# zeromq/jeromq

Hardware: AMD Instinct MI355X
Metric: CURVE encrypt+MAC GiB/s (device-resident), batched 4 KiB frames, 1/2/4/8 GPU (higher is better)
Workload: dtype u32; 1 GPU; 1M x 4 KiB frames, seal (configs[1]); frames_per_gpu=1048576, payload_bytes_per_gpu=4294967296, parallelism=shard1

## Files before the change

### jeromq_amd/build.py

```python
import os
import shutil
import struct
import subprocess
import sys
import tempfile
from concurrent.futures import ThreadPoolExecutor

HERE = os.path.dirname(os.path.abspath(__file__))
ROOT = os.path.dirname(HERE)
CSRC = os.path.join(HERE, "csrc")
PRODUCT_LIB = os.path.join(HERE, "libcurvezmq_mi355x.so")
LIB = os.environ.get("CZ_LIB_OUT", PRODUCT_LIB)
SOURCES = ["cz_kernels.hip#1", "cz_kernels.hip#2", "cz_kernels.hip#3", "cz_x25519.hip", "cz_host.cpp", "cz_mechanism.cpp", "cz_wire.cpp", "cz_engine.cpp", "cz_handshake.cpp", "cz_curve_hs.cpp", "cz_hs_parse.cpp", "cz_acceptor.cpp", "cz_connector.cpp"]
HEADERS = ["cz_accept.h", "cz_accept_kernels.h", "cz_connect.h", "cz_connect_kernels.h", "cz_hs_batch.h", "cz_hs_dev.h",
           "cz_hs_records.h", "cz_hs_parse.h", "cz_device.h", "cz_fe25519.h", "cz_diag.h", "cz_dispatch.h", "cz_internal.h", "cz_launch.h", "cz_salsa_lazy.h", "cz_salsa_tail.h", "cz_session.h", os.path.join("..", "..", "include", "curvezmq_mi355x.h")]
ARCH = os.environ.get("CZ_OFFLOAD_ARCH", "gfx950")
LLVM_BIN = "/opt/rocm/lib/llvm/bin"
BUNDLE_MAGIC = b"__CLANG_OFFLOAD_BUNDLE__"


class IsaHazardError(RuntimeError):
    pass


class ProductFlagsError(ValueError):
    """Extra compile flags (A/B variants, wrong-output diagnostics) asked for the product library."""


def compile_flags(lib, extra_env=None):
    raw = os.environ.get("CZ_EXTRA_FLAGS", "") if extra_env is None else extra_env
    extra = raw.split()
    product = os.path.realpath(lib) == os.path.realpath(PRODUCT_LIB)
    if product and extra:
        raise ProductFlagsError(f"CZ_EXTRA_FLAGS={raw!r} refused for the product library {PRODUCT_LIB}: "
                                "A/B builds set CZ_LIB_OUT to another path")
    common = [f"--offload-arch={ARCH}", "-O3", "-std=c++17", "-fPIC", "-Wall"]
    return common + (["-DCZ_PRODUCT_BUILD"] if product else extra)


def _stale(lib=LIB, sources=SOURCES):
    if not os.path.exists(lib):
        return True
    t = os.path.getmtime(lib)
    return any(os.path.getmtime(os.path.join(CSRC, f.split("#")[0])) > t for f in list(sources) + HEADERS)


def device_code_objects(so_path, arch=ARCH):
    with tempfile.TemporaryDirectory() as td:
        fb = os.path.join(td, "fatbin")
        subprocess.run([os.path.join(LLVM_BIN, "llvm-objcopy"), "--dump-section", f".hip_fatbin={fb}", so_path,
                        os.path.join(td, "discard")], check=True, capture_output=True)
        data = open(fb, "rb").read()
    cos, i = [], data.find(BUNDLE_MAGIC)
    while i >= 0:
        (n,) = struct.unpack_from("<Q", data, i + len(BUNDLE_MAGIC))
        p = i + len(BUNDLE_MAGIC) + 8
        for _ in range(n):
            off, size, tlen = struct.unpack_from("<QQQ", data, p)
            triple = data[p + 24:p + 24 + tlen].decode()
            p += 24 + tlen
            if triple.endswith("--" + arch) and size:
                cos.append(data[i + off:i + off + size])
        i = data.find(BUNDLE_MAGIC, i + 1)
    return cos


def _elf_functions(co):
    (shoff,) = struct.unpack_from("<Q", co, 0x28)
    shentsize, shnum = struct.unpack_from("<HH", co, 0x3A)
    secs = [struct.unpack_from("<IIQQQQIIQQ", co, shoff + k * shentsize) for k in range(shnum)]
    out = []
    for sec in secs:
        if sec[1] != 2:
            continue
        strtab = secs[sec[6]]
        for k in range(sec[5] // 24):
            name_off, info, _, shndx, value, size = struct.unpack_from("<IBBHQQ", co, sec[4] + 24 * k)
            if info & 0xF != 2 or not size or shndx >= len(secs):
                continue
            end = co.index(b"\0", strtab[4] + name_off)
            name = co[strtab[4] + name_off:end].decode()
            text = secs[shndx]
            start = text[4] + (value - text[3])
            out.append((name, bytes(co[start:start + size])))
    return out


def kernel_code_sha256(so_path, kernels, arch=ARCH):
    import hashlib
    funcs = [f for co in device_code_objects(so_path, arch) for f in _elf_functions(co)]
    names = [n for n, _ in funcs]
    filt = shutil.which("c++filt") or shutil.which("llvm-cxxfilt")
    dem = subprocess.run([filt], input="\n".join(names), capture_output=True, text=True, check=True).stdout.split("\n")
    code = {}
    for (n, b), d in zip(funcs, dem):
        d = d.replace("(anonymous namespace)::", "")
        code.setdefault(d.split("(")[0].replace("void ", "", 1).strip(), b)
    h = hashlib.sha256()
    for k in sorted(kernels):
        if k not in code:
            return None
        h.update(k.encode() + b"\0" + code[k])
    return h.hexdigest()


def disassemble(code_object, arch=ARCH):
    with tempfile.NamedTemporaryFile(suffix=".co") as f:
        f.write(code_object)
        f.flush()
        out = subprocess.run([os.path.join(LLVM_BIN, "llvm-objdump"), "-d", f"--mcpu={arch}", f.name],
                             check=True, capture_output=True, text=True).stdout
    lines = []
    for ln in out.splitlines():
        ln = ln.split("//")[0].rstrip()
        if ln.strip() and not ln.endswith(":") and not ln.startswith(("Disassembly", "/")):
            lines.append(ln)
    return "\n".join(lines)


def isa_gate(so_path, arch=ARCH):
    sys.path.insert(0, os.path.join(ROOT, "tools"))
    from isa_store_hazard import scan
    cos = device_code_objects(so_path, arch)
    if not cos:
        raise IsaHazardError(f"{so_path}: no {arch} code object found to scan")
    total, hits = 0, []
    for co in cos:
        text = disassemble(co, arch)
        total += text.count("\n") + 1
        d, s, r = scan(text)
        hits += [("store data rewritten at distance 1", x) for x in d]
        hits += [("VALU-written SGPR read by VMEM within 5 states", x) for x in s]
        hits += [("wide buffer store with a register soffset", x) for x in r]
    if hits:
        raise IsaHazardError(f"{so_path}: {len(hits)} VMEM store hazard(s) in the {arch} ISA, "
                             f"library not installed; first: {hits[:3]}")
    return len(cos), total


def build_library(force=False, verbose=True, sources=None, lib=None, src_dir=None, jobs=None):
    sources = list(sources or SOURCES)
    lib = lib or LIB
    src_dir = src_dir or CSRC
    compile_flags(lib)
    if not force and src_dir == CSRC and not _stale(lib, sources):
        return lib
    hipcc = os.environ.get("HIPCC", "/opt/rocm/bin/hipcc")
    common = compile_flags(lib)
    objdir = tempfile.mkdtemp(prefix="cz_build_")
    try:
        def compile_one(entry):
            f, _, part = entry.partition("#")
            obj = os.path.join(objdir, os.path.splitext(f)[0] + (f"_{part}" if part else "") + ".o")
            cmd = [hipcc] + common + ([f"-DCZ_KPART={part}"] if part else []) + ["-c", "-o", obj, os.path.join(src_dir, f)]
            if verbose:
                print(" ".join(cmd), file=sys.stderr)
            r = subprocess.run(cmd, cwd=src_dir, capture_output=True, text=True)
            if r.returncode:
                errs = [ln for ln in r.stderr.splitlines() if "error" in ln][:20]
                print("\n".join(errs), file=sys.stderr)
                raise subprocess.CalledProcessError(r.returncode, cmd, r.stdout, r.stderr)
            return obj
        order = sorted(sources, key=lambda f: -os.path.getsize(os.path.join(src_dir, f.split("#")[0])))
        with ThreadPoolExecutor(max_workers=jobs or min(len(order), os.cpu_count() or 4, 8)) as ex:
            objs = list(ex.map(compile_one, order))
        tmp = f"{lib}.{os.getpid()}.tmp"
        subprocess.check_call([hipcc, f"--offload-arch={ARCH}", "-shared", "-fPIC", "-o", tmp] + objs, cwd=src_dir)
        try:
            n_co, n_ins = isa_gate(tmp)
        except Exception:
            os.unlink(tmp)
            raise
        if verbose:
            print(f"isa gate: {n_co} {ARCH} code objects, {n_ins} instructions, 0 store hazards", file=sys.stderr)
        os.replace(tmp, lib)
    finally:
        shutil.rmtree(objdir, ignore_errors=True)
    return lib


JNI_DIR = os.path.join(ROOT, "jni")
JNI_BENCH = os.path.join(ROOT, "tools", "bin", "jni_bench")
JNI_WRAPPED = ("cz_box_afternm", "cz_box_open_afternm", "cz_secretbox", "cz_secretbox_open", "cz_box_beforenm", "cz_box",
               "cz_box_open", "cz_box_keypair", "cz_engine_add_conn")


def build_jni_bench(lib=PRODUCT_LIB, out=JNI_BENCH):
    os.makedirs(os.path.dirname(out), exist_ok=True)
    rel = os.path.relpath(os.path.dirname(lib), os.path.dirname(out))
    cmd = ["gcc", "-std=c11", "-O2", "-Wall", "-Wextra", "-Werror", "-DCZ_JNI_MIN", "-I" + JNI_DIR,
           "-I" + os.path.join(ROOT, "include"), os.path.join(JNI_DIR, "jni_bench.c"),
           os.path.join(JNI_DIR, "curvezmq_jni.c"), os.path.join(JNI_DIR, "fake_jni_env.c"),
           "-L" + os.path.dirname(lib), "-lcurvezmq_mi355x", "-Wl,-rpath,$ORIGIN/" + rel,
           "-Wl," + ",".join("--wrap=" + f for f in JNI_WRAPPED), "-o", out]
    subprocess.check_call(cmd)
    return out


if __name__ == "__main__":
    build_library(force="--force" in sys.argv)
    print(LIB)
```

### jeromq_amd/csrc/cz_device.h

```cpp
#pragma once
#include <hip/hip_runtime.h>
#include <stdint.h>

#include "cz_salsa_lazy.h"
#include "cz_salsa_tail.h"

namespace cz {

typedef uint32_t u32;
typedef uint64_t u64;

constexpr u32 SIGMA0 = 0x61707865u, SIGMA1 = 0x3320646eu, SIGMA2 = 0x79622d32u, SIGMA3 = 0x6b206574u;

__device__ __forceinline__ u32 rotl(u32 v, int c) { return __builtin_amdgcn_alignbit(v, v, 32 - c); }

__device__ __forceinline__ void qr(u32 &a, u32 &b, u32 &c, u32 &d)
{
    b ^= rotl(a + d, 7);
    c ^= rotl(b + a, 9);
    d ^= rotl(c + b, 13);
    a ^= rotl(d + c, 18);
}

__device__ __forceinline__ void col_round(u32 x[16])
{
    qr(x[0], x[4], x[8], x[12]);
    qr(x[5], x[9], x[13], x[1]);
    qr(x[10], x[14], x[2], x[6]);
    qr(x[15], x[3], x[7], x[11]);
}

__device__ __forceinline__ void row_round(u32 x[16])
{
    qr(x[0], x[1], x[2], x[3]);
    qr(x[5], x[6], x[7], x[4]);
    qr(x[10], x[11], x[8], x[9]);
    qr(x[15], x[12], x[13], x[14]);
}

template <int C>
__device__ __forceinline__ u32 srotl(u32 v)
{
    u32 r, t;
    asm("s_lshl_b32 %0, %2, %3\n\ts_lshr_b32 %1, %2, %4\n\ts_or_b32 %0, %0, %1"
        : "=&s"(r), "=&s"(t)
        : "s"(v), "i"(C), "i"(32 - C)
        : "scc");
    return r;
}

struct SalsaFrame {
    u32 w[16];
};

__device__ __forceinline__ SalsaFrame salsa_frame(const u32 k[8], u32 n0, u32 n1)
{
    u32 x[16] = {SIGMA0, k[0], k[1], k[2], k[3], SIGMA1, n0, n1, 0u, 0u, SIGMA2, k[4], k[5], k[6], k[7], SIGMA3};
    x[9] ^= srotl<7>(x[5] + x[1]);   x[13] ^= srotl<9>(x[9] + x[5]);
    x[1] ^= srotl<13>(x[13] + x[9]); x[5] ^= srotl<18>(x[1] + x[13]);
    x[14] ^= srotl<7>(x[10] + x[6]); x[2] ^= srotl<9>(x[14] + x[10]);
    x[6] ^= srotl<13>(x[2] + x[14]); x[10] ^= srotl<18>(x[6] + x[2]);
    x[3] ^= srotl<7>(x[15] + x[11]); x[7] ^= srotl<9>(x[3] + x[15]);
    x[11] ^= rotl(x[7] + x[3], 13);  x[15] ^= rotl(x[11] + x[7], 18);
    SalsaFrame f;
#pragma unroll
    for (int i = 0; i < 16; i++)
        f.w[i] = x[i];
    return f;
}

__device__ __forceinline__ void rounds12_frame(u32 x[16], const SalsaFrame &f, u32 c0, const u32 k[8])
{
#pragma unroll
    for (int i = 0; i < 16; i++)
        x[i] = f.w[i];
    x[0] = SIGMA0; x[4] = k[3]; x[8] = c0; x[12] = k[5];
    x[4] ^= srotl<7>(x[0] + x[12]);  x[8] ^= srotl<9>(x[4] + x[0]);
    x[12] ^= srotl<13>(x[8] + x[4]); x[0] ^= srotl<18>(x[12] + x[8]);
    x[1] ^= srotl<7>(x[0] + x[3]);   x[2] ^= srotl<9>(x[1] + x[0]);
    x[3] ^= srotl<13>(x[2] + x[1]);  x[0] ^= srotl<18>(x[3] + x[2]);
    x[6] ^= srotl<7>(x[5] + x[4]);   x[7] ^= srotl<9>(x[6] + x[5]);
    x[4] ^= rotl(x[7] + x[6], 13);   x[5] ^= rotl(x[4] + x[7], 18);
    x[11] ^= rotl(x[10] + x[9], 7);  x[8] ^= rotl(x[11] + x[10], 9);
    x[9] ^= rotl(x[8] + x[11], 13);  x[10] ^= rotl(x[9] + x[8], 18);
    x[12] ^= rotl(x[15] + x[14], 7); x[13] ^= rotl(x[12] + x[15], 9);
    x[14] ^= rotl(x[13] + x[12], 13); x[15] ^= rotl(x[14] + x[13], 18);
}

static_assert(CZ_LAZY_FIRST_ROUND == 3, "rounds_lazy runs rounds 1-2 in C");
template <bool R12 = false>
__device__ __forceinline__ void rounds_lazy(u32 x[16], u32 d[16])
{
    if constexpr (!R12) {
        col_round(x);
        row_round(x);
    }
    u32 t0, t1, t2, t3;
    asm(CZ_SALSA_LAZY_ASM
        : "+v"(x[0]), "+v"(x[1]), "+v"(x[2]), "+v"(x[3]), "+v"(x[4]), "+v"(x[5]), "+v"(x[6]), "+v"(x[7]),
          "+v"(x[8]), "+v"(x[9]), "+v"(x[10]), "+v"(x[11]), "+v"(x[12]), "+v"(x[13]), "+v"(x[14]), "+v"(x[15]),
          "=&v"(d[0]), "=&v"(d[1]), "=&v"(d[2]), "=&v"(d[3]), "=&v"(d[4]), "=&v"(d[5]), "=&v"(d[6]), "=&v"(d[7]),
          "=&v"(d[8]), "=&v"(d[9]), "=&v"(d[10]), "=&v"(d[11]), "=&v"(d[12]), "=&v"(d[13]), "=&v"(d[14]),
          "=&v"(d[15]), "=&v"(t0), "=&v"(t1), "=&v"(t2), "=&v"(t3));
}

__device__ __forceinline__ constexpr bool lazy_pending(int k) { return (CZ_LAZY_PENDING >> k) & 1u; }

__device__ __forceinline__ void rounds_eager(u32 x[16])
{
#pragma unroll
    for (int i = 0; i < 10; i++) {
        col_round(x);
        row_round(x);
    }
}

template <bool LAZY = true>
__device__ __forceinline__ void salsa20_block(u32 x[16], const u32 k[8], u32 n0, u32 n1, u32 c0, u32 c1)
{
    const u32 in[16] = {SIGMA0, k[0], k[1], k[2], k[3], SIGMA1, n0, n1, c0, c1, SIGMA2, k[4], k[5], k[6], k[7], SIGMA3};
#pragma unroll
    for (int i = 0; i < 16; i++)
        x[i] = in[i];
    if constexpr (LAZY) {
        u32 d[16];
        rounds_lazy(x, d);
#pragma unroll
        for (int i = 0; i < 16; i++)
            x[i] = lazy_pending(i) ? ((x[i] ^ d[i]) + in[i]) : (x[i] + in[i]);
    } else {
        rounds_eager(x);
#pragma unroll
        for (int i = 0; i < 16; i++)
            x[i] += in[i];
    }
}

__device__ __forceinline__ void salsa20_block_frame(u32 x[16], const SalsaFrame &f, const u32 k[8], u32 n0, u32 n1,
                                                    u32 c0)
{
    const u32 in[16] = {SIGMA0, k[0], k[1], k[2], k[3], SIGMA1, n0, n1, c0, 0u, SIGMA2, k[4], k[5], k[6], k[7], SIGMA3};
    u32 d[16];
    rounds12_frame(x, f, c0, k);
    rounds_lazy<true>(x, d);
#pragma unroll
    for (int i = 0; i < 16; i++)
        x[i] = lazy_pending(i) ? ((x[i] ^ d[i]) + in[i]) : (x[i] + in[i]);
}

__device__ __forceinline__ void tail_lazy(u32 x[16], u32 d[16])
{
    u32 t0, t1, t2, t3;
    asm(CZ_SALSA_TAIL_ASM
        : "+v"(x[0]), "+v"(x[1]), "+v"(x[2]), "+v"(x[3]), "+v"(x[4]), "+v"(x[5]), "+v"(x[6]), "+v"(x[7]),
          "+v"(x[8]), "+v"(x[9]), "+v"(x[10]), "+v"(x[11]), "+v"(x[12]), "+v"(x[13]), "+v"(x[14]), "+v"(x[15]),
          "=&v"(d[0]), "=&v"(d[1]), "=&v"(d[2]), "=&v"(d[3]), "=&v"(d[4]), "=&v"(d[5]), "=&v"(d[6]), "=&v"(d[7]),
          "=&v"(d[8]), "=&v"(d[9]), "=&v"(d[10]), "=&v"(d[11]), "=&v"(d[12]), "=&v"(d[13]), "=&v"(d[14]),
          "=&v"(d[15]), "=&v"(t0), "=&v"(t1), "=&v"(t2), "=&v"(t3));
}
static_assert(CZ_SALSA_TAIL_WORDS == 4, "tail blocks use keystream words 0..3");

template <bool LAZY = true>
__device__ __forceinline__ void salsa20_block_w03(u32 x[16], const u32 k[8], u32 n0, u32 n1, u32 c0, u32 c1)
{
    const u32 in[16] = {SIGMA0, k[0], k[1], k[2], k[3], SIGMA1, n0, n1, c0, c1, SIGMA2, k[4], k[5], k[6], k[7], SIGMA3};
#pragma unroll
    for (int i = 0; i < 16; i++)
        x[i] = in[i];
    if constexpr (LAZY) {
        u32 d[16];
        col_round(x);
        row_round(x);
        tail_lazy(x, d);
#pragma unroll
        for (int i = 0; i < 4; i++)
            x[i] = lazy_pending(i) ? ((x[i] ^ d[i]) + in[i]) : (x[i] + in[i]);
    } else {
        rounds_eager(x);
#pragma unroll
        for (int i = 0; i < 4; i++)
            x[i] += in[i];
    }
}

__device__ __forceinline__ void salsa20_block_frame_w03(u32 x[16], const SalsaFrame &f, const u32 k[8], u32 n0, u32 n1,
                                                        u32 c0)
{
    const u32 in[4] = {SIGMA0, k[0], k[1], k[2]};
    u32 d[16];
    rounds12_frame(x, f, c0, k);
    tail_lazy(x, d);
#pragma unroll
    for (int i = 0; i < 4; i++)
        x[i] = lazy_pending(i) ? ((x[i] ^ d[i]) + in[i]) : (x[i] + in[i]);
    (void)n0, (void)n1;
}

__device__ __forceinline__ void hsalsa20(u32 out[8], const u32 k[8], const u32 in[4])
{
    u32 x[16], d[16];
    x[0] = SIGMA0; x[1] = k[0]; x[2] = k[1]; x[3] = k[2];
    x[4] = k[3]; x[5] = SIGMA1; x[6] = in[0]; x[7] = in[1];
    x[8] = in[2]; x[9] = in[3]; x[10] = SIGMA2; x[11] = k[4];
    x[12] = k[5]; x[13] = k[6]; x[14] = k[7]; x[15] = SIGMA3;
    rounds_lazy(x, d);
    constexpr int w[8] = {0, 5, 10, 15, 6, 7, 8, 9};
#pragma unroll
    for (int i = 0; i < 8; i++)
        out[i] = lazy_pending(w[i]) ? (x[w[i]] ^ d[w[i]]) : x[w[i]];
}

struct Poly {
    u32 h0, h1, h2, h3, h4;
    u32 r0, r1, r2, r3;
    u32 s1, s2, s3;
    u32 p0, p1, p2, p3;
};

__device__ __forceinline__ void poly_init(Poly &P, u32 k0, u32 k1, u32 k2, u32 k3, u32 k4, u32 k5, u32 k6, u32 k7)
{
    P.r0 = k0 & 0x0fffffffu;
    P.r1 = k1 & 0x0ffffffcu;
    P.r2 = k2 & 0x0ffffffcu;
    P.r3 = k3 & 0x0ffffffcu;
    P.s1 = P.r1 + (P.r1 >> 2);
    P.s2 = P.r2 + (P.r2 >> 2);
    P.s3 = P.r3 + (P.r3 >> 2);
    P.p0 = k4; P.p1 = k5; P.p2 = k6; P.p3 = k7;
    P.h0 = P.h1 = P.h2 = P.h3 = P.h4 = 0;
}

__device__ __forceinline__ u32 addc(u32 a, u32 b, u32 cin, u32 &cout)
{
    return __builtin_addc(a, b, cin, &cout);
}

__device__ __forceinline__ u64 mad64(u32 a, u32 b, u64 c) { return (u64)a * b + c; }

template <bool CIN = false>
__device__ __forceinline__ void poly_block(Poly &P, u32 m0, u32 m1, u32 m2, u32 m3, u32 hibit)
{
    u32 c;
    const u32 h0 = addc(P.h0, m0, 0u, c);
    const u32 h1 = addc(P.h1, m1, c, c);
    const u32 h2 = addc(P.h2, m2, c, c);
    const u32 h3 = addc(P.h3, m3, c, c);
    const u32 h4 = P.h4 + c + hibit;

    const u64 d0 = mad64(h3, P.s1, mad64(h2, P.s2, mad64(h1, P.s3, mad64(h0, P.r0, 0))));
    const u64 d1 = mad64(h4, P.s1, mad64(h3, P.s2, mad64(h2, P.s3, mad64(h1, P.r0, mad64(h0, P.r1, 0)))));
    const u64 d2 = mad64(h4, P.s2, mad64(h3, P.s3, mad64(h2, P.r0, mad64(h1, P.r1, mad64(h0, P.r2, 0)))));
    const u64 d3 = mad64(h4, P.s3, mad64(h3, P.r0, mad64(h2, P.r1, mad64(h1, P.r2, mad64(h0, P.r3, 0)))));
    const u32 h4r = h4 * P.r0;

    const u32 x = (u32)(d3 >> 32) + h4r;
    const u32 q = x >> 2;
    u32 k;
    asm("v_lshl_add_u32 %0, %1, 2, %1" : "=v"(k) : "v"(q));
    if constexpr (CIN) {
        u32 a0 = (u32)d0, a1 = (u32)d1, a2 = (u32)d2, a3 = (u32)d3, a4 = x & 3u;
        asm("v_add_co_u32 %0, vcc, %0, %5\n\ts_nop 1\n\t"
            "v_addc_co_u32 %1, vcc, %1, %6, vcc\n\ts_nop 1\n\t"
            "v_addc_co_u32 %2, vcc, %2, %7, vcc\n\ts_nop 1\n\t"
            "v_addc_co_u32 %3, vcc, %3, %8, vcc\n\ts_nop 1\n\t"
            "v_addc_co_u32 %4, vcc, 0, %4, vcc"
            : "+v"(a0), "+v"(a1), "+v"(a2), "+v"(a3), "+v"(a4)
            : "v"(k), "v"((u32)(d0 >> 32)), "v"((u32)(d1 >> 32)), "v"((u32)(d2 >> 32))
            : "vcc");
        P.h0 = a0; P.h1 = a1; P.h2 = a2; P.h3 = a3; P.h4 = a4;
    } else {
        P.h0 = addc((u32)d0, k, 0u, c);
        P.h1 = addc((u32)d1, (u32)(d0 >> 32), c, c);
        P.h2 = addc((u32)d2, (u32)(d1 >> 32), c, c);
        P.h3 = addc((u32)d3, (u32)(d2 >> 32), c, c);
        P.h4 = (x & 3u) + c;
    }
}

__device__ __forceinline__ void poly_block_partial(Poly &P, u32 m0, u32 m1, u32 m2, u32 m3, u32 len)
{
    u32 m[4] = {m0, m1, m2, m3};
#pragma unroll
    for (int i = 0; i < 4; i++) {
        int rel = (int)len - 4 * i;
        u32 keep = rel >= 4 ? 0xffffffffu : (rel <= 0 ? 0u : ((1u << (8 * rel)) - 1u));
        u32 one = (rel >= 0 && rel < 4) ? (1u << (8 * rel)) : 0u;
        m[i] = (m[i] & keep) | one;
    }
    poly_block(P, m[0], m[1], m[2], m[3], 0u);
}

__device__ __forceinline__ void poly_finish(const Poly &P, u32 tag[4])
{
    u32 h0 = P.h0, h1 = P.h1, h2 = P.h2, h3 = P.h3, h4 = P.h4;
    u64 t;
    u32 c = (h4 >> 2) * 5u;
    h4 &= 3u;
    t = (u64)h0 + c; h0 = (u32)t;
    t = (u64)h1 + (t >> 32); h1 = (u32)t;
    t = (u64)h2 + (t >> 32); h2 = (u32)t;
    t = (u64)h3 + (t >> 32); h3 = (u32)t;
    h4 += (u32)(t >> 32);
    t = (u64)h0 + 5u; u32 g0 = (u32)t;
    t = (u64)h1 + (t >> 32); u32 g1 = (u32)t;
    t = (u64)h2 + (t >> 32); u32 g2 = (u32)t;
    t = (u64)h3 + (t >> 32); u32 g3 = (u32)t;
    u32 g4 = h4 + (u32)(t >> 32);
    bool ge = (g4 >> 2) != 0;
    h0 = ge ? g0 : h0; h1 = ge ? g1 : h1; h2 = ge ? g2 : h2; h3 = ge ? g3 : h3;
    t = (u64)h0 + P.p0; tag[0] = (u32)t;
    t = (u64)h1 + P.p1 + (t >> 32); tag[1] = (u32)t;
    t = (u64)h2 + P.p2 + (t >> 32); tag[2] = (u32)t;
    t = (u64)h3 + P.p3 + (t >> 32); tag[3] = (u32)t;
}

struct F26 {
    u32 l[5];
};

__device__ __forceinline__ F26 f26_from32(u32 h0, u32 h1, u32 h2, u32 h3, u32 h4)
{
    F26 a;
    a.l[0] = h0 & 0x3ffffffu;
    a.l[1] = ((h0 >> 26) | (h1 << 6)) & 0x3ffffffu;
    a.l[2] = ((h1 >> 20) | (h2 << 12)) & 0x3ffffffu;
    a.l[3] = ((h2 >> 14) | (h3 << 18)) & 0x3ffffffu;
    a.l[4] = (h3 >> 8) | (h4 << 24);
    return a;
}

__device__ __forceinline__ F26 f26_mul(const F26 &a, const F26 &b)
{
    const u32 s1 = b.l[1] * 5u, s2 = b.l[2] * 5u, s3 = b.l[3] * 5u, s4 = b.l[4] * 5u;
    u64 d0 = (u64)a.l[0] * b.l[0] + (u64)a.l[1] * s4 + (u64)a.l[2] * s3 + (u64)a.l[3] * s2 + (u64)a.l[4] * s1;
    u64 d1 = (u64)a.l[0] * b.l[1] + (u64)a.l[1] * b.l[0] + (u64)a.l[2] * s4 + (u64)a.l[3] * s3 + (u64)a.l[4] * s2;
    u64 d2 = (u64)a.l[0] * b.l[2] + (u64)a.l[1] * b.l[1] + (u64)a.l[2] * b.l[0] + (u64)a.l[3] * s4 + (u64)a.l[4] * s3;
    u64 d3 = (u64)a.l[0] * b.l[3] + (u64)a.l[1] * b.l[2] + (u64)a.l[2] * b.l[1] + (u64)a.l[3] * b.l[0] + (u64)a.l[4] * s4;
    u64 d4 = (u64)a.l[0] * b.l[4] + (u64)a.l[1] * b.l[3] + (u64)a.l[2] * b.l[2] + (u64)a.l[3] * b.l[1] + (u64)a.l[4] * b.l[0];
    F26 r;
    d1 += d0 >> 26; r.l[0] = (u32)d0 & 0x3ffffffu;
    d2 += d1 >> 26; r.l[1] = (u32)d1 & 0x3ffffffu;
    d3 += d2 >> 26; r.l[2] = (u32)d2 & 0x3ffffffu;
    d4 += d3 >> 26; r.l[3] = (u32)d3 & 0x3ffffffu;
    u64 c = d4 >> 26; r.l[4] = (u32)d4 & 0x3ffffffu;
    u64 t = (u64)r.l[0] + c * 5u;
    r.l[0] = (u32)t & 0x3ffffffu;
    r.l[1] += (u32)(t >> 26);
    return r;
}

__device__ __forceinline__ F26 f26_add(const F26 &a, const F26 &b)
{
    F26 r;
    u32 c = 0;
#pragma unroll
    for (int i = 0; i < 5; i++) {
        u32 v = a.l[i] + b.l[i] + c;
        r.l[i] = v & 0x3ffffffu;
        c = v >> 26;
    }
    u32 t = r.l[0] + c * 5u;
    r.l[0] = t & 0x3ffffffu;
    r.l[1] += t >> 26;
    return r;
}

__device__ __forceinline__ F26 f26_pow(const F26 &r, u32 e)
{
    if (e == 0u)
        return F26{{1u, 0u, 0u, 0u, 0u}};
    F26 acc = r, base = r;
    bool have = false;
    for (u32 bit = 0; e >> bit; bit++) {
        if (bit)
            base = f26_mul(base, base);
        if ((e >> bit) & 1u) {
            acc = have ? f26_mul(acc, base) : base;
            have = true;
        }
    }
    return acc;
}

__device__ __forceinline__ void f26_to32(const F26 &a, u32 &h0, u32 &h1, u32 &h2, u32 &h3, u32 &h4)
{
    u32 l0 = a.l[0], l1 = a.l[1], l2 = a.l[2], l3 = a.l[3], l4 = a.l[4], c;
    c = l1 >> 26; l1 &= 0x3ffffffu;
    l2 += c; c = l2 >> 26; l2 &= 0x3ffffffu;
    l3 += c; c = l3 >> 26; l3 &= 0x3ffffffu;
    l4 += c; c = l4 >> 26; l4 &= 0x3ffffffu;
    l0 += c * 5u; c = l0 >> 26; l0 &= 0x3ffffffu;
    l1 += c;
    h0 = l0 | (l1 << 26);
    h1 = (l1 >> 6) | (l2 << 20);
    h2 = (l2 >> 12) | (l3 << 14);
    h3 = (l3 >> 18) | (l4 << 8);
    h4 = l4 >> 24;
}

__device__ __forceinline__ u32 bswap32(u32 v) { return __builtin_bswap32(v); }

__device__ __forceinline__ void counter_nonce(u64 counter, u32 &n0, u32 &n1)
{
    n0 = bswap32((u32)(counter >> 32));
    n1 = bswap32((u32)counter);
}

}
```

### jeromq_amd/csrc/cz_kernels.hip

```cpp
#include <hip/hip_runtime.h>
#include <stdint.h>

#include <type_traits>

#include "cz_device.h"
#include "cz_diag.h"
#include "cz_dispatch.h"
#include "cz_launch.h"
#include "cz_session.h"
#include "../../include/curvezmq_mi355x.h"

#ifndef CZ_KPART
#define CZ_KPART 0
#endif
#define CZ_KPART_HAS(n) (CZ_KPART == 0 || CZ_KPART == (n))

using namespace cz;
using namespace czd;

namespace {

constexpr u32 HDR0 = 0x53454d07u, HDR1 = 0x45474153u;

#ifdef CZ_SEAL_WAVES_PER_EU
// ... 134 lines not shown
        for (u32 i = 0; i < lim; i++)
            w[i >> 2] |= (u32)p[i] << (8 * (i & 3));
        return V4{w[0], w[1], w[2], w[3]};
    }
}

template <bool AL>
__device__ __forceinline__ u32 ld32(const uint8_t *__restrict__ p)
{
    if constexpr (AL)
        return *reinterpret_cast<const u32 *>(p);
    else
        return (u32)p[0] | ((u32)p[1] << 8) | ((u32)p[2] << 16) | ((u32)p[3] << 24);
}

template <bool AL>
__device__ __forceinline__ V4 ld16f(const uint8_t *__restrict__ p)
{
    if constexpr (AL) {
        uint4 v = *reinterpret_cast<const uint4 *>(p);
        return V4{v.x, v.y, v.z, v.w};
    } else {
        return ld16<false>(p, 16);
    }
}

template <bool AL>
__device__ __forceinline__ V4 ld16f_in(const uint8_t *__restrict__ p)
{
    return ld16f<AL>(p);
}
__device__ __forceinline__ V4 ld16f_8(const uint8_t *__restrict__ p)
{
    const uint2 a = reinterpret_cast<const uint2 *>(p)[0], b = reinterpret_cast<const uint2 *>(p)[1];
    return V4{a.x, a.y, b.x, b.y};
}
__device__ __forceinline__ V4 ld16_8(const uint8_t *__restrict__ p, u64 avail)
{
    if (avail == 0)
        return zero4();
    const uint2 a = reinterpret_cast<const uint2 *>(p)[0];
    const uint2 b = avail > 8u ? reinterpret_cast<const uint2 *>(p)[1] : make_uint2(0u, 0u);
    return V4{a.x, a.y, b.x, b.y};
}

template <bool AL>
__device__ __forceinline__ void st16(uint8_t *__restrict__ p, u32 a, u32 b, u32 c, u32 d)
{
    if constexpr (AL) {
        *reinterpret_cast<uint4 *>(p) = make_uint4(a, b, c, d);
    } else {
        reinterpret_cast<U16ua *>(p)->v = make_uint4(a, b, c, d);
    }
}

__device__ __forceinline__ void st_bytes(uint8_t *__restrict__ p, u32 a, u32 b, u32 c, u32 d, u32 nb)
{
    st_range16(p, make_uint4(a, b, c, d), 0u, nb);
}

__device__ __forceinline__ u32 funnel(u32 hi, u32 lo, u32 sh) { return __builtin_amdgcn_alignbyte(hi, lo, sh); }

__device__ __forceinline__ void mask_chunk(u32 D[16], u32 valid)
{
#pragma unroll
    for (int k = 0; k < 16; k++) {
        int rel = (int)valid - 4 * k;
        u32 keep = rel >= 4 ? 0xffffffffu : (rel <= 0 ? 0u : ((1u << (8 * rel)) - 1u));
        D[k] &= keep;
    }
}

template <bool AL>
struct EmitDirect {
    static constexpr bool cooperative = false;
    uint8_t *dst;
    u32 total;

    __device__ __forceinline__ void emit(u32 q, const u32 D[16])
    {
        const u32 base = 64u * q;
        uint8_t *p = dst + base;
        if (base + 64u <= total) {
            st16<AL>(p, D[0], D[1], D[2], D[3]);
            st16<AL>(p + 16, D[4], D[5], D[6], D[7]);
            st16<AL>(p + 32, D[8], D[9], D[10], D[11]);
            st16<AL>(p + 48, D[12], D[13], D[14], D[15]);
        } else {
#pragma unroll
            for (int c = 0; c < 4; c++) {
                u32 s = base + 16u * c;
                if (s < total) {
                    u32 nb = total - s;
                    if (nb >= 16)
                        st16<AL>(dst + s, D[4 * c], D[4 * c + 1], D[4 * c + 2], D[4 * c + 3]);
                    else
                        st_bytes(dst + s, D[4 * c], D[4 * c + 1], D[4 * c + 2], D[4 * c + 3], nb);
                }
            }
        }
    }
    __device__ __forceinline__ void emit_full(u32 q, const u32 D[16])
    {
        uint8_t *p = dst + 64u * q;
        st16<AL>(p, D[0], D[1], D[2], D[3]);
        st16<AL>(p + 16, D[4], D[5], D[6], D[7]);
        st16<AL>(p + 32, D[8], D[9], D[10], D[11]);
        st16<AL>(p + 48, D[12], D[13], D[14], D[15]);
    }
    __device__ __forceinline__ void tag(const u32 t[4]) { st16<AL>(dst + 16, t[0], t[1], t[2], t[3]); }
    __device__ __forceinline__ void finish() {}
    __device__ __forceinline__ void close(bool bad)
    {
        if (bad)
            poison();
    }
    __device__ void poison()
    {
        for (u32 o = 0; o < total; o += 16) {
            u32 nb = total - o < 16 ? total - o : 16;
            if (nb == 16)
                st16<AL>(dst + o, 0u, 0u, 0u, 0u);
            else
                st_bytes(dst + o, 0u, 0u, 0u, 0u, nb);
        }
    }
};

template <int CP>
struct EmitLinesT {
    static constexpr bool cooperative = true;
    uint4 *lds;
    uint8_t *wbase;
    uint8_t *mine;
    u64 stride;
    u32 lane, total, last_q;
    bool tag_slot;
    uint4 *hold;
    u32 head[12];
    u32 tagw[4];

    __device__ __forceinline__ void flush(u32 line, bool whole = false)
    {
        const u32 c = lane & 7u;
        const u32 r = lane >> 3;
        const u64 lb = uniform64((u64)(uintptr_t)wbase) + 128ull * line;
        const u32 voff = r * (u32)stride + 16u * c;
        const u32 step = 8u * (u32)stride;
        const bool skip = tag_slot && line == 0 && !whole;
        asm volatile("s_waitcnt lgkmcnt(0)" ::: "memory");
#pragma unroll
        for (u32 j = 0; j < 8; j++) {
            const u32 F = 8u * j + r;
            uint4 v = lds[F * 8u + (c ^ (F & 7u))];
            if (!skip)
                buf_store16<CP>(lb + (u64)(j * step), voff, v);
        }
    }
    __device__ __forceinline__ void emit(u32 q, const u32 Din[16])
    {
        u32 D[16];
#pragma unroll
        for (int k = 0; k < 16; k++)
            D[k] = Din[k];
        if (64u * q + 64u > total)
            mask_chunk(D, total > 64u * q ? total - 64u * q : 0u);
        emit_full(q, D);
    }
    __device__ __forceinline__ void emit_full(u32 q, const u32 D[16])
    {
        if (tag_slot && q == 0u) {
#pragma unroll
            for (int k = 0; k < 4; k++)
                head[k] = D[k];
#pragma unroll
            for (int k = 0; k < 8; k++)
                head[4 + k] = D[8 + k];
        }
        if (tag_slot && q == 1u) {
#pragma unroll
            for (u32 c = 0; c < 4; c++)
                hold[lane * 4u + c] = make_uint4(D[4 * c], D[4 * c + 1], D[4 * c + 2], D[4 * c + 3]);
        }
        const u32 h = q & 1u;
        const u32 sw = lane & 7u;
#pragma unroll
        for (u32 c = 0; c < 4; c++)
            lds[lane * 8u + ((4u * h + c) ^ sw)] = make_uint4(D[4 * c], D[4 * c + 1], D[4 * c + 2], D[4 * c + 3]);
        if (h)
            flush(q >> 1);
        last_q = q;
    }
    __device__ __forceinline__ void tag(const u32 t[4])
    {
#pragma unroll
        for (int k = 0; k < 4; k++)
            tagw[k] = t[k];
    }
    __device__ __forceinline__ void line0()
    {
        const u32 sw = lane & 7u;
        const bool one = last_q == 0u;
        uint4 b1[4];
#pragma unroll
        for (u32 c = 0; c < 4; c++)
            b1[c] = one ? make_uint4(0u, 0u, 0u, 0u) : hold[lane * 4u + c];
        lds[lane * 8u + (0u ^ sw)] = make_uint4(head[0], head[1], head[2], head[3]);
        lds[lane * 8u + (1u ^ sw)] = make_uint4(tagw[0], tagw[1], tagw[2], tagw[3]);
        lds[lane * 8u + (2u ^ sw)] = make_uint4(head[4], head[5], head[6], head[7]);
        lds[lane * 8u + (3u ^ sw)] = make_uint4(head[8], head[9], head[10], head[11]);
#pragma unroll
        for (u32 c = 0; c < 4; c++)
            lds[lane * 8u + ((4u + c) ^ sw)] = b1[c];
        flush(0, true);
    }
    __device__ __forceinline__ void finish()
    {
        if ((last_q & 1u) == 0) {
            const u32 sw = lane & 7u;
#pragma unroll
            for (u32 c = 4; c < 8; c++)
                lds[lane * 8u + (c ^ sw)] = make_uint4(0u, 0u, 0u, 0u);
            flush(last_q >> 1);
        }
    }
    __device__ __forceinline__ void close(bool bad)
    {
        finish();
        if (tag_slot)
            line0();
        if (bad)
            poison();
    }
    __device__ void poison()
    {
        __threadfence_block();
        for (u32 o = 0; o < total; o += 16)
            *reinterpret_cast<uint4 *>(mine + o) = make_uint4(0u, 0u, 0u, 0u);
    }
};
using EmitLines = EmitLinesT<CZ_OPEN_STORE_CPOL>;
using EmitLinesSeal = EmitLinesT<CZ_SEAL_STORE_CPOL>;


template <int CP>
struct EmitRegionT {
    static constexpr bool cooperative = true;
    uint4 *lds;
    uint8_t *wbase;
    u32 stride, lane, total;

    __device__ __forceinline__ void emit(u32 q, const u32 Din[16])
    {
        u32 D[16];
#pragma unroll
        for (int k = 0; k < 16; k++)
            D[k] = Din[k];
        if (64u * q + 64u > total)
            mask_chunk(D, total > 64u * q ? total - 64u * q : 0u);
        const u32 base = (lane * stride + 64u * q) >> 4;
#pragma unroll
        for (u32 c = 0; c < 4; c++)
            if (64u * q + 16u * c < stride)
                lds[base + c] = make_uint4(D[4 * c], D[4 * c + 1], D[4 * c + 2], D[4 * c + 3]);
    }
    __device__ __forceinline__ void emit_full(u32 q, const u32 D[16])
    {
        const u32 base = (lane * stride + 64u * q) >> 4;
#pragma unroll
        for (u32 c = 0; c < 4; c++)
            lds[base + c] = make_uint4(D[4 * c], D[4 * c + 1], D[4 * c + 2], D[4 * c + 3]);
    }
    __device__ __forceinline__ void tag(const u32 t[4]) { lds[(lane * stride + 16u) >> 4] = make_uint4(t[0], t[1], t[2], t[3]); }
    __device__ __forceinline__ void finish()
    {
        const u32 done = ((total + 63u) & ~63u) < stride ? ((total + 63u) & ~63u) : stride;
        for (u32 o = done; o < stride; o += 16u)
            lds[(lane * stride + o) >> 4] = make_uint4(0u, 0u, 0u, 0u);
        const u32 n16 = (64u * stride) >> 4;
        asm volatile("s_waitcnt lgkmcnt(0)" ::: "memory");
        for (u32 k = lane; k < n16; k += 64u) {
            const uint4 v = lds[k];
            if constexpr (CP == 2)
                __builtin_nontemporal_store(v4u_t{v.x, v.y, v.z, v.w}, reinterpret_cast<v4u_t *>(wbase) + k);
            else
                reinterpret_cast<uint4 *>(wbase)[k] = v;
        }
    }
    __device__ __forceinline__ void close(bool bad)
    {
        if (bad)
            poison();
        finish();
    }
    __device__ void poison()
    {
        for (u32 o = 0; o < stride; o += 16u)
            lds[(lane * stride + o) >> 4] = make_uint4(0u, 0u, 0u, 0u);
    }
};
using EmitRegion = EmitRegionT<CZ_OPEN_STORE_CPOL>;
using EmitRegionSeal = EmitRegionT<CZ_SEAL_STORE_CPOL == 2 ? 2 : 0>;

template <int MODE, bool AL, class EM, bool PAIR = false, bool UN0 = false, bool LAZY = true, int INA = 16>
__device__ __forceinline__ void seal_frame(const uint8_t *__restrict__ in0, u32 n, u32 flags, u64 counter,
                                           const u32 key[8], EM &em)
{
    static_assert(INA == 16 || (MODE == MODE_ZMQ && AL), "INA 8/1: MESSAGE seal on the AL code paths");
    const u32 ina_a = INA == 1 ? (u32)(uintptr_t)in0 & 3u : 0u;
    const u32 ina_d = (4u - ina_a) & 3u;
    const uint8_t *__restrict__ in = in0 + ina_d;
    const u32 sh = ina_a ? ina_a - 1u : 3u;
    u32 pm1 = flags << 24;
    if constexpr (INA == 1) {
        if (ina_a) {
            const u32 r = *reinterpret_cast<const u32 *>(in0 - ina_a);
            pm1 = (r & ~(0xffu << (8u * sh))) | (flags << (8u * sh));
        }
    }
    auto ldF = [&](const uint8_t *p) -> V4 {
        if constexpr (INA == 16) {
            return ld16f_in<AL>(p);
        } else {
            const uint4 r = *reinterpret_cast<const u4_a4 *>(p);
            return V4{r.x, r.y, r.z, r.w};
        }
    };
    auto ldP = [&](const uint8_t *p, u64 avail) -> V4 {
        if constexpr (INA == 16)
            return ld16<AL>(p, avail);
        else
            return avail >= 16u ? ldF(p) : ld16<false>(p, avail);
    };
    const u32 mlen = (MODE == MODE_ZMQ || MODE == MODE_BOX) ? n + 33u : n;
    const u32 nfull = mlen >> 6;
    const u32 tailv = mlen & 63u;
    const u64 inlen = MODE == MODE_BOX ? (u64)mlen : (n > ina_d ? (u64)(n - ina_d) : 0ull);
    u32 n0, n1;
    counter_nonce(counter, n0, n1);
    if constexpr (UN0)
        n0 = __builtin_amdgcn_readfirstlane(n0);

    [[maybe_unused]] SalsaFrame sf{};
    if constexpr (UN0 && LAZY)
        sf = salsa_frame(key, n0, n1);
    auto ksblock = [&](u32 *xs, u32 c0, u32 c1) {
        if constexpr (UN0 && LAZY)
            salsa20_block_frame(xs, sf, key, n0, n1, c0);
        else
            salsa20_block<LAZY>(xs, key, n0, n1, c0, c1);
    };
    auto ksblock_w03 = [&](u32 *xs, u32 c0) {
        if constexpr (UN0 && LAZY)
            salsa20_block_frame_w03(xs, sf, key, n0, n1, c0);
        else
            salsa20_block_w03<LAZY>(xs, key, n0, n1, c0, 0u);
    };
    u32 x[16], C[16];
    ksblock(x, 0u, 0u);
    Poly P;
    poly_init(P, x[0], x[1], x[2], x[3], x[4], x[5], x[6], x[7]);

    auto zmq_block_win = [&](u32 blk, auto win, auto steady) {
        ksblock(x, blk, 0u);
#pragma unroll
        for (int k = 0; k < 16; k++)
            C[k] = funnel(win(k + 1), win(k), sh) ^ x[k];
        constexpr bool STEADY = decltype(steady)::value;
        poly_block<STEADY>(P, C[0], C[1], C[2], C[3], 1u);
        poly_block<STEADY>(P, C[4], C[5], C[6], C[7], 1u);
        poly_block<STEADY>(P, C[8], C[9], C[10], C[11], 1u);
        poly_block<STEADY>(P, C[12], C[13], C[14], C[15], 1u);
        if constexpr (STEADY)
            emit_steady(em, blk, C);
        else
            em.emit_full(blk, C);
    };
    auto zmq_full_block = [&](u32 blk, const u32 *W) {
        zmq_block_win(blk, [&](int q) { return W[q]; }, std::false_type{});
    };

    [[maybe_unused]] auto box_full_block = [&](u32 blk, const u32 *W) {
        ksblock(x, blk, 0u);
#pragma unroll
        for (int k = 0; k < 16; k++)
            C[k] = W[k] ^ x[k];
        poly_block(P, C[0], C[1], C[2], C[3], 1u);
        poly_block(P, C[4], C[5], C[6], C[7], 1u);
        poly_block(P, C[8], C[9], C[10], C[11], 1u);
        poly_block(P, C[12], C[13], C[14], C[15], 1u);
        em.emit_full(blk, C);
    };

    u32 carry = 0;
    u32 blk = 1;
    if constexpr (MODE == MODE_BOX && AL && PAIR) {
        u32 L[32];
#pragma unroll
        for (int c = 2; c < 8; c++) {
            V4 v = ld16<AL>(in + 16 * c, inlen > 16u * c ? inlen - 16u * c : 0);
            L[4 * c] = v.x; L[4 * c + 1] = v.y; L[4 * c + 2] = v.z; L[4 * c + 3] = v.w;
        }
#pragma unroll
        for (int k = 8; k < 16; k++)
            C[k] = L[k] ^ x[k];
        C[0] = HDR0; C[1] = HDR1; C[2] = n0; C[3] = n1;
        C[4] = C[5] = C[6] = C[7] = 0u;
        if (nfull >= 1) {
            poly_block(P, C[8], C[9], C[10], C[11], 1u);
            poly_block(P, C[12], C[13], C[14], C[15], 1u);
        } else {
            const u32 nb = mlen - 32u;
            if (nb >= 16u) {
                poly_block(P, C[8], C[9], C[10], C[11], 1u);
                if (nb > 16u)
                    poly_block_partial(P, C[12], C[13], C[14], C[15], nb - 16u);
            } else {
                poly_block_partial(P, C[8], C[9], C[10], C[11], nb);
            }
        }
        em.emit(0, C);
        if (nfull >= 2) {
            box_full_block(1, L + 16);
            for (u32 k = 1; 2u * k + 1u < nfull; k++) {
                const uint8_t *src = in + 128u * k;
#pragma unroll
                for (int c = 0; c < 8; c++) {
                    V4 v = ld16f_in<AL>(src + 16 * c);
                    L[4 * c] = v.x; L[4 * c + 1] = v.y; L[4 * c + 2] = v.z; L[4 * c + 3] = v.w;
                }
                box_full_block(2u * k, L);
                box_full_block(2u * k + 1u, L + 16);
                blk = 2u * k + 2u;
            }
            if (blk < 2u)
                blk = 2u;
        } else {
            blk = nfull > 1 ? nfull : 1u;
        }
    } else if constexpr (MODE == MODE_ZMQ && AL && PAIR) {
        u32 L[32];
#pragma unroll
        for (int c = 0; c < 8; c++) {
            V4 v = ldP(in + 16 * c, inlen > 16u * c ? inlen - 16u * c : 0);
            L[4 * c] = v.x; L[4 * c + 1] = v.y; L[4 * c + 2] = v.z; L[4 * c + 3] = v.w;
        }
        {
            C[8] = funnel(L[0], pm1, sh) ^ x[8];
#pragma unroll
            for (int k = 9; k < 16; k++)
                C[k] = funnel(L[k - 8], L[k - 9], sh) ^ x[k];
            C[0] = HDR0; C[1] = HDR1; C[2] = n0; C[3] = n1;
            C[4] = C[5] = C[6] = C[7] = 0u;
            if (nfull >= 1) {
                poly_block(P, C[8], C[9], C[10], C[11], 1u);
                poly_block(P, C[12], C[13], C[14], C[15], 1u);
            } else {
                u32 nb = mlen - 32u;
                if (nb >= 16u) {
                    poly_block(P, C[8], C[9], C[10], C[11], 1u);
                    if (nb > 16u)
                        poly_block_partial(P, C[12], C[13], C[14], C[15], nb - 16u);
                } else {
                    poly_block_partial(P, C[8], C[9], C[10], C[11], nb);
                }
            }
            em.emit(0, C);
        }
        carry = L[7];
        if (nfull >= 2) {
            auto load_chunks = [&](u32 k, u32 *D, auto nch) {
                const uint8_t *src = in + 128u * k;
#pragma unroll
                for (int c = 0; c < decltype(nch)::value; c++) {
                    V4 v = ldF(src + 16 * c);
                    D[4 * c] = v.x; D[4 * c + 1] = v.y; D[4 * c + 2] = v.z; D[4 * c + 3] = v.w;
                }
            };
            auto pair = [&](u32 k, const u32 *Cur, const u32 *Prev) {
                zmq_block_win(2u * k, [&](int q) { return q < 9 ? Prev[23 + q] : Cur[q - 9]; }, std::true_type{});
                zmq_block_win(2u * k + 1u, [&](int q) { return Cur[7 + q]; }, std::true_type{});
            };
            zmq_full_block(1, L + 7);
            const u32 kend = nfull >> 1;
            const u32 klines = INA == 1 ? (n > 3u ? (n - 3u) >> 7 : 0u) : (u32)(inlen >> 7);
            const u32 kst = kend < klines ? kend : klines;
            u32 M[32];
            u32 k = 1;
            for (; k < kst; k++) {
                load_chunks(k, M, std::integral_constant<int, 8>{});
                pair(k, M, L);
#pragma unroll
                for (int q = 23; q < 32; q++)
                    L[q] = M[q];
            }
            if (k < kend) {
                load_chunks(k, M, std::integral_constant<int, 6>{});
                pair(k, M, L);
                L[23] = M[23];
                k++;
            }
            blk = 2u * k;
            carry = L[23];
        } else {
            blk = nfull > 1 ? nfull : 1u;
        }
    } else {
        if constexpr (MODE == MODE_ZMQ) {
            V4 a = ldP(in, inlen);
            V4 b = ldP(in + 16, inlen > 16 ? inlen - 16 : 0);
            u32 W[9] = {pm1, a.x, a.y, a.z, a.w, b.x, b.y, b.z, b.w};
#pragma unroll
            for (int k = 8; k < 16; k++)
                C[k] = funnel(W[k - 7], W[k - 8], sh) ^ x[k];
            carry = b.w;
            C[0] = HDR0; C[1] = HDR1; C[2] = n0; C[3] = n1;
        } else {
            V4 a = ld16<AL>(in + 32, inlen > 32 ? inlen - 32 : 0);
            V4 b = ld16<AL>(in + 48, inlen > 48 ? inlen - 48 : 0);
            C[8] = a.x ^ x[8]; C[9] = a.y ^ x[9]; C[10] = a.z ^ x[10]; C[11] = a.w ^ x[11];
            C[12] = b.x ^ x[12]; C[13] = b.y ^ x[13]; C[14] = b.z ^ x[14]; C[15] = b.w ^ x[15];
            carry = 0;
            if constexpr (MODE == MODE_BOX) {
                C[0] = HDR0; C[1] = HDR1; C[2] = n0; C[3] = n1;
            } else {
                C[0] = C[1] = C[2] = C[3] = 0u;
            }
        }
        C[4] = C[5] = C[6] = C[7] = 0u;
        if (nfull >= 1) {
            poly_block(P, C[8], C[9], C[10], C[11], 1u);
            poly_block(P, C[12], C[13], C[14], C[15], 1u);
        } else {
            if (mlen > 32u) {
                u32 nb = mlen - 32u;
                if (nb >= 16u) {
                    poly_block(P, C[8], C[9], C[10], C[11], 1u);
                    if (nb > 16u)
                        poly_block_partial(P, C[12], C[13], C[14], C[15], nb - 16u);
                } else {
                    poly_block_partial(P, C[8], C[9], C[10], C[11], nb);
                }
            }
        }
        em.emit(0, C);
    }

    for (; blk < nfull; blk++) {
        V4 q0, q1, q2, q3;
        if constexpr (MODE == MODE_ZMQ) {
            const uint8_t *src = in + 64u * blk - 32u;
            q0 = ldF(src);
            q1 = ldF(src + 16);
            q2 = ldF(src + 32);
            q3 = ldP(src + 48, inlen - (64u * blk + 16u));
            u32 W[17] = {carry, q0.x, q0.y, q0.z, q0.w, q1.x, q1.y, q1.z, q1.w,
                         q2.x, q2.y, q2.z, q2.w, q3.x, q3.y, q3.z, q3.w};
            zmq_full_block(blk, W);
            carry = q3.w;
        } else {
            const uint8_t *src = in + 64u * blk;
            q0 = ld16f_in<AL>(src);
            q1 = ld16f_in<AL>(src + 16);
            q2 = ld16f_in<AL>(src + 32);
            q3 = ld16f_in<AL>(src + 48);
            ksblock(x, blk, 0u);
            u32 W[16] = {q0.x, q0.y, q0.z, q0.w, q1.x, q1.y, q1.z, q1.w,
                         q2.x, q2.y, q2.z, q2.w, q3.x, q3.y, q3.z, q3.w};
#pragma unroll
            for (int k = 0; k < 16; k++)
                C[k] = W[k] ^ x[k];
            poly_block(P, C[0], C[1], C[2], C[3], 1u);
            poly_block(P, C[4], C[5], C[6], C[7], 1u);
            poly_block(P, C[8], C[9], C[10], C[11], 1u);
            poly_block(P, C[12], C[13], C[14], C[15], 1u);
            em.emit_full(blk, C);
        }
    }

    if (tailv != 0 && tailv <= 16u && nfull >= 1) {
        const u32 blk = nfull;
        const long o = (MODE == MODE_ZMQ) ? (long)(64u * blk) - 32 : (long)(64u * blk);
        const V4 q = ldP(in + o, (o >= 0 && (u64)o < inlen) ? inlen - (u64)o : 0);
        ksblock_w03(x, blk);
        if constexpr (MODE == MODE_ZMQ) {
            C[0] = funnel(q.x, carry, sh) ^ x[0];
            C[1] = funnel(q.y, q.x, sh) ^ x[1];
            C[2] = funnel(q.z, q.y, sh) ^ x[2];
            C[3] = funnel(q.w, q.z, sh) ^ x[3];
        } else {
            C[0] = q.x ^ x[0]; C[1] = q.y ^ x[1]; C[2] = q.z ^ x[2]; C[3] = q.w ^ x[3];
        }
#pragma unroll
        for (int k = 4; k < 16; k++)
            C[k] = 0u;
        if (tailv == 16u)
            poly_block(P, C[0], C[1], C[2], C[3], 1u);
        else
            poly_block_partial(P, C[0], C[1], C[2], C[3], tailv);
        em.emit(blk, C);
    } else if (tailv != 0 && nfull >= 1) {
        const u32 blk = nfull;
        V4 q[4];
#pragma unroll
        for (int c = 0; c < 4; c++) {
            long o = (MODE == MODE_ZMQ) ? (long)(64u * blk) - 32 + 16 * c : (long)(64u * blk) + 16 * c;
            u64 avail = (o >= 0 && (u64)o < inlen) ? inlen - (u64)o : 0;
            q[c] = ldP(in + o, avail);
        }
        ksblock(x, blk, 0u);
        u32 W[16] = {q[0].x, q[0].y, q[0].z, q[0].w, q[1].x, q[1].y, q[1].z, q[1].w,
                     q[2].x, q[2].y, q[2].z, q[2].w, q[3].x, q[3].y, q[3].z, q[3].w};
        if constexpr (MODE == MODE_ZMQ) {
            C[0] = funnel(W[0], carry, sh) ^ x[0];
#pragma unroll
            for (int k = 1; k < 16; k++)
                C[k] = funnel(W[k], W[k - 1], sh) ^ x[k];
        } else {
#pragma unroll
            for (int k = 0; k < 16; k++)
                C[k] = W[k] ^ x[k];
        }
#pragma unroll
        for (int j = 0; j < 4; j++) {
            u32 s = 16u * j;
            if (s < tailv) {
                u32 nb = tailv - s;
                if (nb >= 16)
                    poly_block(P, C[4 * j], C[4 * j + 1], C[4 * j + 2], C[4 * j + 3], 1u);
                else
                    poly_block_partial(P, C[4 * j], C[4 * j + 1], C[4 * j + 2], C[4 * j + 3], nb);
            }
        }
        em.emit(blk, C);
    }

    u32 tag[4];
    poly_finish(P, tag);
    em.tag(tag);
    em.close(false);
}

template <int S, int BASE>
__device__ __forceinline__ void carry_window_s(u32 C[16], const u32 Cur[32], const u32 Nxt[32], u32 ina)
{
#pragma unroll
    for (int q = 0; q < 16; q++) {
        const int lo = BASE + q + S, hi = lo + 1;
        const u32 vlo = lo < 32 ? Cur[lo & 31] : Nxt[(lo - 32) & 31];
        const u32 vhi = hi < 32 ? Cur[hi & 31] : Nxt[(hi - 32) & 31];
        C[q] = funnel(vhi, vlo, ina);
    }
}
template <int BASE>
__device__ __forceinline__ void carry_window(u32 C[16], const u32 Cur[32], const u32 Nxt[32], u32 s, u32 ina)
{
    switch (s) {
#define CZ_CW(S) case S: carry_window_s<S, BASE>(C, Cur, Nxt, ina); break;
        CZ_CW(0) CZ_CW(1) CZ_CW(2) CZ_CW(3) CZ_CW(4) CZ_CW(5) CZ_CW(6) CZ_CW(7)
        CZ_CW(8) CZ_CW(9) CZ_CW(10) CZ_CW(11) CZ_CW(12) CZ_CW(13) CZ_CW(14) CZ_CW(15)
        CZ_CW(16) CZ_CW(17) CZ_CW(18) CZ_CW(19) CZ_CW(20) CZ_CW(21) CZ_CW(22) CZ_CW(23)
        CZ_CW(24) CZ_CW(25) CZ_CW(26) CZ_CW(27) CZ_CW(28) CZ_CW(29) CZ_CW(30)
        default: carry_window_s<31, BASE>(C, Cur, Nxt, ina); break;
#undef CZ_CW
    }
}

template <int MODE, bool AL, class EM, bool PAIR = false, bool UN0 = false, bool LAZY = true, int INA = 16,
          bool CARRY = false>
__device__ __forceinline__ u32 open_frame(const uint8_t *__restrict__ in, u32 size, const u32 key[8],
                                          bool check_floor, long long floor, u32 *flags_out, u64 *nonce_out,
                                          u64 nacl_counter, EM &em)
{
    static_assert(INA == 16 || (AL && (INA == 8 || INA == 1)), "INA 8/1 take the AL code paths");
    const u32 ina = INA == 1 ? (u32)(uintptr_t)in & 3u : 0u;
    const uint8_t *in4 = in - ina;
    auto LF = [&](u32 off) -> V4 {
        if constexpr (INA == 16) {
            return ld16f<AL>(in + off);
        } else {
            const uint4 r = *reinterpret_cast<const u4_a4 *>(in4 + off);
            if constexpr (INA == 8)
                return V4{r.x, r.y, r.z, r.w};
            const u32 r4 = ina ? *reinterpret_cast<const u32 *>(in4 + off + 16) : 0u;
            return V4{funnel(r.y, r.x, ina), funnel(r.z, r.y, ina), funnel(r.w, r.z, ina), funnel(r4, r.w, ina)};
        }
    };
    auto LP = [&](u32 off, u64 avail) -> V4 {
        if constexpr (INA == 16)
            return ld16<AL>(in + off, avail);
        else
            return avail >= 16u ? LF(off) : ld16<false>(in + off, avail);
    };
    constexpr bool COOP = EM::cooperative;
    u32 early = CZ_STATUS_OK;
    u32 n0, n1;
    if constexpr (MODE == MODE_ZMQ) {
        V4 h = LP(0, size);
        if (size < 8u || h.x != HDR0 || (h.y & 0x00ffffffu) != (HDR1 & 0x00ffffffu))
            early = CZ_STATUS_COMMAND;
        else if (size < 33u)
            early = CZ_STATUS_MALFORMED;
        n0 = h.z;
        n1 = h.w;
        if (early == CZ_STATUS_OK) {
            u64 nonce = ((u64)bswap32(n0) << 32) | (u64)bswap32(n1);
            *nonce_out = nonce;
            if (check_floor && (long long)nonce <= floor)
                early = CZ_STATUS_SEQUENCE;
        }
    } else {
        if (size < 32u)
            early = CZ_STATUS_MALFORMED;
        counter_nonce(nacl_counter, n0, n1);
    }
    if (early != CZ_STATUS_OK && (!COOP || size < 33u))
        return early;
    const bool dead = early != CZ_STATUS_OK;
    if constexpr (UN0)
        n0 = __builtin_amdgcn_readfirstlane(n0);
    [[maybe_unused]] SalsaFrame sf{};
    if constexpr (UN0 && LAZY)
        sf = salsa_frame(key, n0, n1);
    auto ksblock = [&](u32 *xs, u32 c0, u32 c1) {
        if constexpr (UN0 && LAZY)
            salsa20_block_frame(xs, sf, key, n0, n1, c0);
        else
            salsa20_block<LAZY>(xs, key, n0, n1, c0, c1);
    };
    auto ksblock_w03 = [&](u32 *xs, u32 c0) {
        if constexpr (UN0 && LAZY)
            salsa20_block_frame_w03(xs, sf, key, n0, n1, c0);
        else
            salsa20_block_w03<LAZY>(xs, key, n0, n1, c0, 0u);
    };

    const u32 mlen = size;
    const u32 nblk = (mlen + 63u) >> 6;
    const u32 nfull = mlen >> 6;
    const u32 nout = (MODE == MODE_ZMQ) ? size - 33u : size;

    auto emit_open = [&](u32 q, u32 D[16], bool full) {
        if (COOP && dead) {
#pragma unroll
            for (int k = 0; k < 16; k++)
                D[k] = 0u;
        }
        if (full)
            em.emit_full(q, D);
        else
            em.emit(q, D);
    };

    constexpr bool EARLY0 = PAIR && AL && MODE == MODE_ZMQ;
    const bool early0 = EARLY0 && nfull >= 2;
    [[maybe_unused]] V4 e_tin{}, e_a{}, e_b{};
    [[maybe_unused]] u32 L1[16];
    if constexpr (EARLY0) {
        if (early0) {
            e_tin = LF(16);
            e_a = LF(32);
            e_b = LF(48);
#pragma unroll
            for (int c = 0; c < 4; c++) {
                V4 v = LF(64 + 16 * c);
                L1[4 * c] = v.x; L1[4 * c + 1] = v.y; L1[4 * c + 2] = v.z; L1[4 * c + 3] = v.w;
            }
        }
    }
    u32 x[16], C[16], X[16];
    ksblock(x, 0u, 0u);
    Poly P;
    poly_init(P, x[0], x[1], x[2], x[3], x[4], x[5], x[6], x[7]);
    V4 tin = early0 ? e_tin : LP(16, size - 16u);

    u32 K[8];

    {
        V4 a = early0 ? e_a : LP(32, size > 32 ? size - 32u : 0);
        V4 b = early0 ? e_b : LP(48, size > 48 ? size - 48u : 0);
        C[8] = a.x; C[9] = a.y; C[10] = a.z; C[11] = a.w;
        C[12] = b.x; C[13] = b.y; C[14] = b.z; C[15] = b.w;
        if (nfull >= 1) {
            poly_block(P, C[8], C[9], C[10], C[11], 1u);
            poly_block(P, C[12], C[13], C[14], C[15], 1u);
        } else if (mlen > 32u) {
            u32 nb = mlen - 32u;
            if (nb >= 16u) {
                poly_block(P, C[8], C[9], C[10], C[11], 1u);
                if (nb > 16u)
                    poly_block_partial(P, C[12], C[13], C[14], C[15], nb - 16u);
            } else {
                poly_block_partial(P, C[8], C[9], C[10], C[11], nb);
            }
        }
#pragma unroll
        for (int k = 8; k < 16; k++)
            X[k] = C[k] ^ x[k];
        if constexpr (MODE == MODE_ZMQ) {
            *flags_out = X[8] & 0xffu;
#pragma unroll
            for (int k = 0; k < 8; k++)
                K[k] = X[8 + k];
        } else {
#pragma unroll
            for (int k = 0; k < 8; k++)
                X[k] = 0u;
            emit_open(0, X, false);
        }
    }

    auto open_block_f = [&](u32 blk, bool full, bool drain, const u32 *Rf, auto &&fillC) {
        if (!full && mlen - 64u * blk <= 16u)
            ksblock_w03(x, blk);
        else
            ksblock(x, blk, 0u);
        if (Rf) {
            __builtin_amdgcn_sched_barrier(0);
#pragma unroll
            for (int q = 0; q < 16; q++)
                C[q] = funnel(Rf[q + 1], Rf[q], ina);
        }
        fillC();
        if (full) {
            poly_block(P, C[0], C[1], C[2], C[3], 1u);
            poly_block(P, C[4], C[5], C[6], C[7], 1u);
            poly_block(P, C[8], C[9], C[10], C[11], 1u);
            poly_block(P, C[12], C[13], C[14], C[15], 1u);
        } else {
            const u32 tailv = mlen - 64u * blk;
#pragma unroll
            for (int j = 0; j < 4; j++) {
                u32 s = 16u * j;
                if (s < tailv) {
                    u32 nb = tailv - s;
                    if (nb >= 16)
                        poly_block(P, C[4 * j], C[4 * j + 1], C[4 * j + 2], C[4 * j + 3], 1u);
                    else
                        poly_block_partial(P, C[4 * j], C[4 * j + 1], C[4 * j + 2], C[4 * j + 3], nb);
                }
            }
        }
#pragma unroll
        for (int k = 0; k < 16; k++)
            X[k] = C[k] ^ x[k];
        if constexpr (MODE == MODE_ZMQ) {
            u32 O[16];
            u32 E[17] = {K[0], K[1], K[2], K[3], K[4], K[5], K[6], K[7], X[0], X[1], X[2], X[3], X[4], X[5], X[6],
                         X[7], X[8]};
#pragma unroll
            for (int t = 0; t < 16; t++)
                O[t] = funnel(E[t + 1], E[t], 1);
            if (drain)
                __builtin_amdgcn_s_waitcnt(0x0f70);
            emit_open(blk - 1, O, full);
#pragma unroll
            for (int k = 0; k < 8; k++)
                K[k] = X[8 + k];
        } else {
            emit_open(blk, X, full);
        }
    };
    auto open_block = [&](u32 blk, bool full, bool drain = false, const u32 *Rf = nullptr) {
        open_block_f(blk, full, drain, Rf, [] {});
    };

    u32 blk = 1;
    if constexpr (PAIR && AL) {
        if (nfull >= 2) {
#pragma unroll
            for (int k = 0; k < 16; k++)
                C[k] = L1[k];
            open_block(1, true);
            blk = 2;
            if constexpr (CARRY) {
                static_assert(INA != 16, "carry-line input is for bodies off 16-byte alignment");
                const uint8_t *lb = reinterpret_cast<const uint8_t *>((uintptr_t)in4 & ~(uintptr_t)127);
                const u32 s = __builtin_amdgcn_readfirstlane(((u32)(uintptr_t)in4 & 127u) >> 2);
                u32 Cur[32], Nxt[32];
                auto load_line = [&](u32 *D, const uint8_t *p) {
#pragma unroll
                    for (int c = 0; c < 8; c++) {
                        const uint4 v = *reinterpret_cast<const uint4 *>(p + 16 * c);
                        D[4 * c] = v.x; D[4 * c + 1] = v.y; D[4 * c + 2] = v.z; D[4 * c + 3] = v.w;
                    }
                };
                load_line(Cur, lb + 128);
                for (u32 k = 1; 2u * k + 1u < nfull; k++) {
                    load_line(Nxt, lb + 128u * (k + 1u));
                    __builtin_amdgcn_sched_barrier(0);
                    open_block_f(2u * k, true, true, nullptr, [&] {
                        __builtin_amdgcn_sched_barrier(0);
                        carry_window<0>(C, Cur, Nxt, s, ina);
                    });
                    open_block_f(2u * k + 1u, true, false, nullptr, [&] {
                        __builtin_amdgcn_sched_barrier(0);
                        carry_window<16>(C, Cur, Nxt, s, ina);
                    });
#pragma unroll
                    for (int q = 0; q < 32; q++)
                        Cur[q] = Nxt[q];
                    blk = 2u * k + 2u;
                }
            }
            for (u32 k = 1; !CARRY && 2u * k + 1u < nfull; k++) {
                u32 M[32];
                if constexpr (INA == 1) {
                    const uint8_t *src4 = in4 + 128u * k;
                    u32 R[33];
#pragma unroll
                    for (int c = 0; c < 8; c++) {
                        const uint4 v = *reinterpret_cast<const u4_a4 *>(src4 + 16 * c);
                        R[4 * c] = v.x; R[4 * c + 1] = v.y; R[4 * c + 2] = v.z; R[4 * c + 3] = v.w;
                    }
                    R[32] = ina ? *reinterpret_cast<const u32 *>(src4 + 128) : 0u;
                    __builtin_amdgcn_sched_barrier(0);
                    open_block(2u * k, true, true, R);
                    open_block(2u * k + 1u, true, false, R + 16);
                    blk = 2u * k + 2u;
                    continue;
                } else {
#pragma unroll
                    for (int c = 0; c < 8; c++) {
                        V4 v = LF(128u * k + 16u * c);
                        M[4 * c] = v.x; M[4 * c + 1] = v.y; M[4 * c + 2] = v.z; M[4 * c + 3] = v.w;
                    }
                }
#pragma unroll
                for (int q = 0; q < 16; q++)
                    C[q] = M[q];
                open_block(2u * k, true, true);
#pragma unroll
                for (int q = 0; q < 16; q++)
                    C[q] = M[16 + q];
                open_block(2u * k + 1u, true);
                blk = 2u * k + 2u;
            }
        }
    }
    for (; blk < nblk; blk++) {
        const uint8_t *src = in + 64u * blk;
        V4 q0, q1, q2, q3;
        const bool full = blk < nfull;
        const u32 o = 64u * blk;
        if (full) {
            q0 = LF(o);
            q1 = LF(o + 16u);
            q2 = LF(o + 32u);
            q3 = LF(o + 48u);
        } else {
            q0 = LP(o, size - o);
            q1 = LP(o + 16u, o + 16u < size ? size - o - 16u : 0);
            q2 = LP(o + 32u, o + 32u < size ? size - o - 32u : 0);
            q3 = LP(o + 48u, o + 48u < size ? size - o - 48u : 0);
        }
        (void)src;
        C[0] = q0.x; C[1] = q0.y; C[2] = q0.z; C[3] = q0.w;
        C[4] = q1.x; C[5] = q1.y; C[6] = q1.z; C[7] = q1.w;
        C[8] = q2.x; C[9] = q2.y; C[10] = q2.z; C[11] = q2.w;
        C[12] = q3.x; C[13] = q3.y; C[14] = q3.z; C[15] = q3.w;
        open_block(blk, full);
    }
    if constexpr (MODE == MODE_ZMQ) {
        if (64u * (nblk - 1u) < nout) {
            u32 O[16];
#pragma unroll
            for (int t = 0; t < 16; t++)
                O[t] = t < 7 ? funnel(K[t + 1], K[t], 1) : (t == 7 ? funnel(0u, K[7], 1) : 0u);
            emit_open(nblk - 1u, O, false);
        }
    }

    u32 tag[4];
    poly_finish(P, tag);
    u32 diff = (tag[0] ^ tin.x) | (tag[1] ^ tin.y) | (tag[2] ^ tin.z) | (tag[3] ^ tin.w);
    const bool bad = dead || diff != 0;
    em.close(bad);
    if (dead)
        return early;
    return diff != 0 ? (u32)CZ_STATUS_CRYPTO : (u32)CZ_STATUS_OK;
}

__device__ __forceinline__ void load_key(const uint8_t *__restrict__ p, u32 k[8])
{
    const uint4 *q = reinterpret_cast<const uint4 *>(p);
    uint4 a = q[0], b = q[1];
    k[0] = a.x; k[1] = a.y; k[2] = a.z; k[3] = a.w;
    k[4] = b.x; k[5] = b.y; k[6] = b.z; k[7] = b.w;
}

__device__ __forceinline__ bool aligned16(const void *a, const void *b)
{
    return (((uintptr_t)a | (uintptr_t)b) & 15u) == 0;
}

__device__ __forceinline__ bool wave_uniform(u32 v)
{
    return __builtin_amdgcn_ballot_w64(v != __builtin_amdgcn_readfirstlane(v)) == 0;
}

__device__ __forceinline__ u64 read_be64(const uint8_t *p)
{
    u64 v = 0;
    for (int b = 0; b < 8; b++)
        v = (v << 8) | p[b];
    return v;
}


__device__ __forceinline__ void st_range16_g(u64 p, uint4 v, u32 a, u32 b)
{
    if (b <= a)
        return;
    u64 lo = ((u64)v.y << 32) | v.x, hi = ((u64)v.w << 32) | v.z;
    if (a >= 8u) {
        lo = hi >> (8u * (a - 8u));
        hi = 0;
    } else if (a) {
        lo = (lo >> (8u * a)) | (hi << (64u - 8u * a));
        hi >>= 8u * a;
    }
    u64 q = p + a;
    const u32 n = b - a;
    if (n == 16u) {
        *reinterpret_cast<g_v4u_ua *>(q) = v4u_t{v.x, v.y, v.z, v.w};
        return;
    }
    if (n & 8u) {
        *reinterpret_cast<g_u64_ua *>(q) = lo;
// ... 640 lines not shown
            if (blk == 0) {
                V4 a = ldP(in, inlen);
                V4 b = ldP(in + 16, inlen > 16 ? inlen - 16 : 0);
                W[8] = carry;
                W[9] = a.x; W[10] = a.y; W[11] = a.z; W[12] = a.w;
                W[13] = b.x; W[14] = b.y; W[15] = b.z; W[16] = b.w;
#pragma unroll
                for (int k = 1; k < 8; k++)
                    W[k] = 0u;
            } else {
                const uint8_t *src = in + 64u * blk - 32u;
                V4 q0, q1, q2, q3;
                if (blk < nfull) {
                    q0 = ldF(src); q1 = ldF(src + 16); q2 = ldF(src + 32);
                    q3 = ldP(src + 48, inlen - (64u * blk + 16u));
                } else {
                    const u64 o = 64u * blk - 32u;
                    q0 = ldP(src, o < inlen ? inlen - o : 0);
                    q1 = ldP(src + 16, o + 16 < inlen ? inlen - o - 16 : 0);
                    q2 = ldP(src + 32, o + 32 < inlen ? inlen - o - 32 : 0);
                    q3 = ldP(src + 48, o + 48 < inlen ? inlen - o - 48 : 0);
                }
                W[1] = q0.x; W[2] = q0.y; W[3] = q0.z; W[4] = q0.w;
                W[5] = q1.x; W[6] = q1.y; W[7] = q1.z; W[8] = q1.w;
                W[9] = q2.x; W[10] = q2.y; W[11] = q2.z; W[12] = q2.w;
                W[13] = q3.x; W[14] = q3.y; W[15] = q3.z; W[16] = q3.w;
            }
            block(blk, W);
            carry = W[16];
            em.emit(q, C);
        }
    }
    if (!rec) {
        u32 tag[4];
        poly_finish(P, tag);
        em.tag(tag);
    }
    em.close(false);
    if (rec) {
        rec[0] = P.h0; rec[1] = P.h1; rec[2] = P.h2; rec[3] = P.h3; rec[4] = P.h4; rec[5] = mpoly;
        if (b0 == 0) {
            rec[8] = P.r0; rec[9] = P.r1; rec[10] = P.r2; rec[11] = P.r3;
            rec[12] = P.p0; rec[13] = P.p1; rec[14] = P.p2; rec[15] = P.p3;
        }
    }
}

__device__ __forceinline__ u32 open_header(const uint8_t *__restrict__ in, u32 size, bool check_floor,
                                           long long floor, u32 &n0, u32 &n1, u64 &nonce)
{
    if (size < 8u)
        return CZ_STATUS_COMMAND;
    V4 h = ld16<false>(in, size);
    if (h.x != HDR0 || (h.y & 0x00ffffffu) != (HDR1 & 0x00ffffffu))
        return CZ_STATUS_COMMAND;
    if (size < 33u)
        return CZ_STATUS_MALFORMED;
    n0 = h.z;
    n1 = h.w;
    nonce = ((u64)bswap32(n0) << 32) | (u64)bswap32(n1);
    if (check_floor && (long long)nonce <= floor)
        return CZ_STATUS_SEQUENCE;
    return CZ_STATUS_OK;
}

struct OpenSeg {
    u32 nblk, nout, cb, ce, bend;
};
__device__ __forceinline__ OpenSeg open_seg_geom(u32 size, u32 b0, u32 b1)
{
    OpenSeg g;
    g.nblk = (size + 63u) >> 6;
    g.nout = size - 33u;
    g.bend = b1 < g.nblk ? b1 : g.nblk;
    g.cb = b0 ? b0 - 1u : 0u;
    g.ce = g.bend == g.nblk ? (g.nout + 63u) >> 6 : g.bend - 1u;
    return g;
}

template <bool AL, class EM, bool AL8 = false, bool ANY = false>
__device__ __forceinline__ u32 open_segment(const uint8_t *__restrict__ in, u32 size, const u32 key[8], u32 n0, u32 n1, u32 b0,
                            u32 b1, u32 *__restrict__ rec, u32 &flags_out, EM &em)
{
    const u32 ina = ANY ? (u32)(uintptr_t)in & 3u : 0u;
    const uint8_t *in4 = in - ina;
    auto ldf = [&](const uint8_t *p) -> V4 {
        if constexpr (ANY) {
            const uint8_t *q = in4 + (p - in);
            const uint4 r = *reinterpret_cast<const u4_a4 *>(q);
            const u32 r4 = ina ? *reinterpret_cast<const u32 *>(q + 16) : 0u;
            return V4{funnel(r.y, r.x, ina), funnel(r.z, r.y, ina), funnel(r.w, r.z, ina), funnel(r4, r.w, ina)};
        } else if constexpr (AL8) {
            return ld16f_8(p);
        } else {
            return ld16f<AL>(p);
        }
    };
    auto ldp = [&](const uint8_t *p, u64 avail) -> V4 {
        if constexpr (ANY)
            return avail >= 16u ? ldf(p) : ld16<false>(p, avail);
        else if constexpr (AL8)
            return ld16_8(p, avail);
        else
            return ld16<AL>(p, avail);
    };
    const OpenSeg g = open_seg_geom(size, b0, b1);
    const u32 mlen = size;
    const u32 nfull = mlen >> 6;
    u32 x[16], X[16], K[8];
    salsa20_block(x, key, n0, n1, 0u, 0u);
    Poly P;
    poly_init(P, x[0], x[1], x[2], x[3], x[4], x[5], x[6], x[7]);
    u32 mpoly = 0;
    if (b0 == 0) {
        V4 a = ldp(in + 32, size > 32 ? size - 32u : 0);
        V4 b = ldp(in + 48, size > 48 ? size - 48u : 0);
        const u32 nb = (mlen < 64u ? mlen : 64u) - 32u;
        if (nb >= 16u) {
            poly_block(P, a.x, a.y, a.z, a.w, 1u);
            mpoly++;
            if (nb >= 32u) {
                poly_block(P, b.x, b.y, b.z, b.w, 1u);
                mpoly++;
            } else if (nb > 16u) {
                poly_block_partial(P, b.x, b.y, b.z, b.w, nb - 16u);
                mpoly++;
            }
        } else if (nb > 0u) {
            poly_block_partial(P, a.x, a.y, a.z, a.w, nb);
            mpoly++;
        }
        K[0] = a.x ^ x[8]; K[1] = a.y ^ x[9]; K[2] = a.z ^ x[10]; K[3] = a.w ^ x[11];
        K[4] = b.x ^ x[12]; K[5] = b.y ^ x[13]; K[6] = b.z ^ x[14]; K[7] = b.w ^ x[15];
        flags_out = K[0] & 0xffu;
    } else {
        salsa20_block(X, key, n0, n1, g.cb, 0u);
        const uint8_t *src = in + 64u * g.cb + 32u;
        V4 a = ldf(src), b = ldf(src + 16);
        K[0] = a.x ^ X[8]; K[1] = a.y ^ X[9]; K[2] = a.z ^ X[10]; K[3] = a.w ^ X[11];
        K[4] = b.x ^ X[12]; K[5] = b.y ^ X[13]; K[6] = b.z ^ X[14]; K[7] = b.w ^ X[15];
    }
    for (u32 q = 0; q < g.ce - g.cb; q++) {
        const u32 blk = g.cb + q + 1u;
        if (blk < g.nblk) {
            const uint8_t *src = in + 64u * blk;
            V4 q0, q1, q2, q3;
            const bool full = blk < nfull;
            if (full) {
                q0 = ldf(src); q1 = ldf(src + 16); q2 = ldf(src + 32); q3 = ldf(src + 48);
            } else {
                const u32 o = 64u * blk;
                q0 = ldp(src, size - o);
                q1 = ldp(src + 16, o + 16u < size ? size - o - 16u : 0);
                q2 = ldp(src + 32, o + 32u < size ? size - o - 32u : 0);
                q3 = ldp(src + 48, o + 48u < size ? size - o - 48u : 0);
            }
            u32 C[16] = {q0.x, q0.y, q0.z, q0.w, q1.x, q1.y, q1.z, q1.w,
                         q2.x, q2.y, q2.z, q2.w, q3.x, q3.y, q3.z, q3.w};
            salsa20_block(x, key, n0, n1, blk, 0u);
            if (full) {
                poly_block(P, C[0], C[1], C[2], C[3], 1u);
                poly_block(P, C[4], C[5], C[6], C[7], 1u);
                poly_block(P, C[8], C[9], C[10], C[11], 1u);
                poly_block(P, C[12], C[13], C[14], C[15], 1u);
                mpoly += 4;
            } else {
                const u32 tailv = mlen - 64u * blk;
#pragma unroll
                for (int j = 0; j < 4; j++) {
                    const u32 s = 16u * j;
                    if (s < tailv) {
                        const u32 nb = tailv - s;
                        if (nb >= 16)
                            poly_block(P, C[4 * j], C[4 * j + 1], C[4 * j + 2], C[4 * j + 3], 1u);
                        else
                            poly_block_partial(P, C[4 * j], C[4 * j + 1], C[4 * j + 2], C[4 * j + 3], nb);
                        mpoly++;
                    }
                }
            }
#pragma unroll
            for (int k = 0; k < 16; k++)
                X[k] = C[k] ^ x[k];
        } else {
#pragma unroll
            for (int k = 0; k < 16; k++)
                X[k] = 0u;
        }
        u32 O[16];
        u32 E[17] = {K[0], K[1], K[2], K[3], K[4], K[5], K[6], K[7], X[0], X[1], X[2], X[3], X[4], X[5], X[6], X[7],
                     X[8]};
#pragma unroll
        for (int t = 0; t < 16; t++)
            O[t] = funnel(E[t + 1], E[t], 1);
        em.emit(q, O);
#pragma unroll
        for (int k = 0; k < 8; k++)
            K[k] = X[8 + k];
    }
    bool bad = false;
    if (!rec) {
        u32 tag[4];
        poly_finish(P, tag);
        V4 tin = ld16<AL>(in + 16, size - 16u);
        bad = ((tag[0] ^ tin.x) | (tag[1] ^ tin.y) | (tag[2] ^ tin.z) | (tag[3] ^ tin.w)) != 0;
    }
    em.close(bad);
    if (!rec)
        return bad ? CZ_STATUS_CRYPTO : CZ_STATUS_OK;
    rec[0] = P.h0; rec[1] = P.h1; rec[2] = P.h2; rec[3] = P.h3; rec[4] = P.h4; rec[5] = mpoly;
    if (b0 == 0) {
        rec[6] = flags_out;
        rec[8] = P.r0; rec[9] = P.r1; rec[10] = P.r2; rec[11] = P.r3;
        rec[12] = P.p0; rec[13] = P.p1; rec[14] = P.p2; rec[15] = P.p3;
    }
    return CZ_STATUS_OK;
}

__device__ __forceinline__ void combine_tag(const u32 *__restrict__ R0, u32 nseg, u32 tag[4])
{
    const F26 r = f26_from32(R0[8], R0[9], R0[10], R0[11], 0u);
    F26 H = f26_from32(R0[0], R0[1], R0[2], R0[3], R0[4]);
    if (nseg > 1u) {
        const u32 *RL = R0 + 16u * (nseg - 1u);
        const u32 m_last = RL[5];
        const u32 m_mid = nseg > 2u ? R0[16 + 5] : m_last;
        const F26 hl = f26_from32(RL[0], RL[1], RL[2], RL[3], RL[4]);
        F26 hn = nseg > 2u ? f26_from32(R0[16], R0[17], R0[18], R0[19], R0[20]) : hl;
        F26 base = r, pm = {{1u, 0u, 0u, 0u, 0u}}, pl = pm;
        for (u32 bit = 0; __builtin_amdgcn_ballot_w64(((m_mid | m_last) >> bit) != 0u) != 0; bit++) {
            if (bit)
                base = f26_mul(base, base);
            if ((m_mid >> bit) & 1u)
                pm = f26_mul(pm, base);
            if ((m_last >> bit) & 1u)
                pl = f26_mul(pl, base);
        }
        for (u32 s = 1; s + 1u < nseg; s++) {
            const u32 *R = R0 + 16u * s;
            const F26 h = hn;
            const u32 m = R[5];
            if (s + 2u < nseg)
                hn = f26_from32(R[16], R[17], R[18], R[19], R[20]);
            F26 pw = pm;
            if (m != m_mid)
                pw = f26_pow(r, m);
            H = f26_add(f26_mul(H, pw), h);
        }
        H = f26_add(f26_mul(H, pl), hl);
    }
    Poly Q;
    if (nseg > 1u) {
        f26_to32(H, Q.h0, Q.h1, Q.h2, Q.h3, Q.h4);
    } else {
        Q.h0 = R0[0]; Q.h1 = R0[1]; Q.h2 = R0[2]; Q.h3 = R0[3]; Q.h4 = R0[4];
    }
    Q.p0 = R0[12]; Q.p1 = R0[13]; Q.p2 = R0[14]; Q.p3 = R0[15];
    poly_finish(Q, tag);
}


template <int ST, bool PAIR, int MODE, int INA>
__device__ __forceinline__ void seal_uniform_body(const uint8_t *__restrict__ in, uint64_t in_stride,
                                                  uint8_t *__restrict__ out, uint64_t out_stride, uint32_t count,
                                                  uint32_t len, const uint8_t *__restrict__ subkey, uint64_t counter0,
                                                  const uint8_t *__restrict__ flags8, int allow_un0)
{
    extern __shared__ uint4 smem[];
    uint32_t i = blockIdx.x * BLOCK + threadIdx.x;
    if constexpr (ST == ST_SHIFT) {
        if (blockIdx.x * BLOCK + BLOCK <= count)
            i = blockIdx.x * BLOCK + class_permute(((uintptr_t)(out + (uint64_t)i * out_stride) & 64u) != 0,
                                                   reinterpret_cast<u32 *>(smem));
    }
    const uint32_t wave_first = (blockIdx.x * BLOCK + threadIdx.x) & ~63u;
    if (wave_first >= count)
        return;
    u32 key[8];
    load_key(subkey, key);
    const bool full_wave = wave_first + 64u <= count;
    const uint8_t *src = in + (uint64_t)i * in_stride;
    uint8_t *dst = out + (uint64_t)i * out_stride;
    const u32 mlen = len + 33u;
    const bool un0 = allow_un0 && wave_uniform((u32)((counter0 + i) >> 32));
    if (ST != ST_DIRECT && full_wave) {
        const u32 fl = (MODE == MODE_ZMQ && flags8) ? flags8[i] : 0u;
        const u32 lane = threadIdx.x & 63u;
        if constexpr (ST == ST_LINES) {
            using EmL = EmitLinesSeal;
            EmL em{smem + (threadIdx.x >> 6) * (LINE_LDS_BYTES / 16), out + (uint64_t)wave_first * out_stride,
                   dst, out_stride, lane, mlen, 0u, true,
                   smem + (WAVES * LINE_LDS_BYTES + (threadIdx.x >> 6) * HOLD_LDS_BYTES) / 16};
            if (un0)
                seal_frame<MODE, true, EmL, PAIR, true, true, INA>(src, len, fl, counter0 + i, key, em);
            else
                seal_frame<MODE, true, EmL, PAIR, false, true, INA>(src, len, fl, counter0 + i, key, em);
        } else if constexpr (ST == ST_SHIFT) {
            EmitShiftLinesUniSeal em{reinterpret_cast<uint8_t *>(smem) + (threadIdx.x >> 6) * SHIFT_LDS_BYTES, dst, lane,
                                 mlen, 0u, 0u};
            em.init(true, true);
            em.init_uniform(i - blockIdx.x * BLOCK, (u32)out_stride, out + (uint64_t)blockIdx.x * BLOCK * out_stride);
            const bool b2b = out_stride == (uint64_t)mlen && (mlen & 63u) != 0u;
            em.init_ext(b2b && i > 0u, b2b && i + 1u < count);
            if (un0 && !em.mixed) {
                if (__builtin_amdgcn_readfirstlane((((u32)(uintptr_t)dst & 64u) == 0u) ? 1u : 0u)) {
                    EmitShiftLinesUniClassSeal<1> ec{em};
                    seal_frame<MODE, true, EmitShiftLinesUniClassSeal<1>, PAIR, true, true, INA>(src, len, fl,
                                                                                               counter0 + i, key, ec);
                } else {
                    EmitShiftLinesUniClassSeal<0> ec{em};
                    seal_frame<MODE, true, EmitShiftLinesUniClassSeal<0>, PAIR, true, true, INA>(src, len, fl,
                                                                                               counter0 + i, key, ec);
                }
            } else if (un0)
                seal_frame<MODE, true, EmitShiftLinesUniSeal, PAIR, true, true, INA>(src, len, fl, counter0 + i, key, em);
            else
                seal_frame<MODE, true, EmitShiftLinesUniSeal, PAIR, false, true, INA>(src, len, fl, counter0 + i, key, em);
        } else {
            const u32 st = (u32)out_stride;
            EmitRegionSeal em{smem + (threadIdx.x >> 6) * ((64u * st) >> 4), out + (uint64_t)wave_first * out_stride, st,
                          lane, mlen};
            if (un0)
                seal_frame<MODE, true, EmitRegionSeal, PAIR, true, true, INA>(src, len, fl, counter0 + i, key, em);
            else
                seal_frame<MODE, true, EmitRegionSeal, PAIR, false, true, INA>(src, len, fl, counter0 + i, key, em);
        }
        return;
    }
    if (i >= count)
        return;
    const u32 fl = (MODE == MODE_ZMQ && flags8) ? flags8[i] : 0u;
    if (aligned16(src, dst)) {
        EmitDirect<true> em{dst, mlen};
        seal_frame<MODE, true, EmitDirect<true>, PAIR>(src, len, fl, counter0 + i, key, em);
    } else if ((((uintptr_t)src) & 15u) == 0) {
        EmitDirect<false> em{dst, mlen};
        seal_frame<MODE, true, EmitDirect<false>, PAIR>(src, len, fl, counter0 + i, key, em);
    } else {
        EmitDirect<false> em{dst, mlen};
        seal_frame<MODE, false>(src, len, fl, counter0 + i, key, em);
    }
    if constexpr (ST == ST_LINES || ST == ST_REGION)
        if (out_stride > mlen)
            zero_bytes(dst + mlen, (u32)(out_stride - mlen));
}

#ifdef CZ_DIAG_CLOCK
constexpr u32 DIAG_CLOCK_WAVES = 1u << 16;
static __device__ uint64_t g_diag_clock[DIAG_CLOCK_WAVES * 4u];
#define CZ_DIAG_CLOCK_BEGIN                                                                                   \
    const uint64_t dc_t0 = __builtin_amdgcn_s_memtime(), dc_r0 = __builtin_amdgcn_s_memrealtime();
#define CZ_DIAG_CLOCK_END                                                                                     \
    {                                                                                                         \
        const uint64_t dc_t1 = __builtin_amdgcn_s_memtime(), dc_r1 = __builtin_amdgcn_s_memrealtime();       \
        const u32 w = blockIdx.x * WAVES + (threadIdx.x >> 6);                                                \
        if ((threadIdx.x & 63u) == 0u && w < DIAG_CLOCK_WAVES) {                                              \
            volatile uint64_t *g = g_diag_clock + 4u * w;                                                     \
            g[0] = dc_t0; g[1] = dc_r0; g[2] = dc_t1; g[3] = dc_r1;                                           \
        }                                                                                                     \
    }
#else
#define CZ_DIAG_CLOCK_BEGIN
#define CZ_DIAG_CLOCK_END
#endif

template <int ST, bool PAIR, int MODE = MODE_ZMQ>
__global__ __launch_bounds__(BLOCK) CZ_OCC CZ_OPEN_UNI_OCC void k_seal_uniform(const uint8_t *__restrict__ in, uint64_t in_stride,
                                                         uint8_t *__restrict__ out, uint64_t out_stride,
                                                         uint32_t count, uint32_t len,
                                                         const uint8_t *__restrict__ subkey, uint64_t counter0,
                                                         const uint8_t *__restrict__ flags8, int allow_un0)
{
    CZ_DIAG_CLOCK_BEGIN
    seal_uniform_body<ST, PAIR, MODE, 16>(in, in_stride, out, out_stride, count, len, subkey, counter0, flags8,
                                          allow_un0);
    CZ_DIAG_CLOCK_END
}

template <int ST, bool PAIR, int INA>
__global__ __launch_bounds__(BLOCK) CZ_OCC CZ_OPEN_UNI_OCC void k_seal_uniform_ina(
    const uint8_t *__restrict__ in, uint64_t in_stride, uint8_t *__restrict__ out, uint64_t out_stride, uint32_t count,
    uint32_t len, const uint8_t *__restrict__ subkey, uint64_t counter0, const uint8_t *__restrict__ flags8,
    int allow_un0)
{
    seal_uniform_body<ST, PAIR, MODE_ZMQ, INA>(in, in_stride, out, out_stride, count, len, subkey, counter0, flags8,
                                               allow_un0);
}

__device__ __forceinline__ const uint8_t *per_lane_ptr(const uint8_t *p)
{
    asm volatile("" : "+v"(p));
    return p;
}
#ifdef CZ_FANOUT_VGPR_PAYLOAD
#define CZ_FANOUT_SRC(p) per_lane_ptr(p)
#else
#define CZ_FANOUT_SRC(p) (p)
#endif
template <int ST, bool PAIR>
__device__ __forceinline__ void seal_fanout_wave(const uint8_t *__restrict__ payload, uint32_t len, uint32_t flags,
                                                 const cz_fanout_sub *__restrict__ subs,
                                                 const uint8_t *__restrict__ subkeys, uint8_t *__restrict__ out,
                                                 uint64_t out_stride, uint32_t count, int owns, uint32_t wave_first,
                                                 bool staged, u32 region_part16)
{
    extern __shared__ uint4 smem[];
    const uint32_t i = wave_first + (threadIdx.x & 63u);
    if (wave_first >= count)
        return;
    const bool full_wave = wave_first + 64u <= count;
    const u32 mlen = len + 33u;
    const u32 fl = flags & 0xffu;
    const uint8_t *src = CZ_FANOUT_SRC(payload);
    if (ST != ST_DIRECT && full_wave && staged) {
        const cz_fanout_sub sb = subs[i];
        u32 key[8];
        load_key(subkeys + 32ull * sb.key_idx, key);
        uint8_t *dst = out + (uint64_t)i * out_stride;
        const u32 lane = threadIdx.x & 63u;
        if constexpr (ST == ST_LINES) {
            using EmL = EmitLinesSeal;
            EmL em{smem + (threadIdx.x >> 6) * (LINE_LDS_BYTES / 16), out + (uint64_t)wave_first * out_stride,
                   dst, out_stride, lane, mlen, 0u, true,
                   smem + (WAVES * LINE_LDS_BYTES + (threadIdx.x >> 6) * HOLD_LDS_BYTES) / 16};
            seal_frame<MODE_ZMQ, true, EmL, PAIR, false, true, 16>(src, len, fl, sb.counter, key, em);
            const u32 body_lines = (mlen + 127u) & ~127u;
            if (out_stride > body_lines)
                zero_bytes(dst + body_lines, (u32)(out_stride - body_lines));
        } else {
            const u32 st = (u32)out_stride;
            EmitRegionSeal em{smem + (threadIdx.x >> 6) * region_part16, out + (uint64_t)wave_first * out_stride, st,
                              lane, mlen};
            seal_frame<MODE_ZMQ, true, EmitRegionSeal, PAIR, false, true, 16>(src, len, fl, sb.counter, key, em);
        }
        return;
    }
    if (i >= count)
        return;
    const cz_fanout_sub sb = subs[i];
    u32 key[8];
    load_key(subkeys + 32ull * sb.key_idx, key);
    uint8_t *dst = out + (uint64_t)i * out_stride;
    if (aligned16(src, dst)) {
        EmitDirect<true> em{dst, mlen};
        seal_frame<MODE_ZMQ, true, EmitDirect<true>, PAIR>(src, len, fl, sb.counter, key, em);
    } else if ((((uintptr_t)src) & 15u) == 0) {
        EmitDirect<false> em{dst, mlen};
        seal_frame<MODE_ZMQ, true, EmitDirect<false>, PAIR>(src, len, fl, sb.counter, key, em);
    } else {
        EmitDirect<false> em{dst, mlen};
        seal_frame<MODE_ZMQ, false>(per_lane_ptr(src), len, fl, sb.counter, key, em);
    }
    if (owns && out_stride > mlen)
        zero_bytes(dst + mlen, (u32)(out_stride - mlen));
}

template <int ST, bool PAIR>
__global__ __launch_bounds__(BLOCK) CZ_OCC CZ_OPEN_UNI_OCC void k_seal_fanout(
    const uint8_t *__restrict__ payload, uint32_t len, uint32_t flags, const cz_fanout_sub *__restrict__ subs,
    const uint8_t *__restrict__ subkeys, uint8_t *__restrict__ out, uint64_t out_stride, uint32_t count, int owns)
{
    seal_fanout_wave<ST, PAIR>(payload, len, flags, subs, subkeys, out, out_stride, count, owns,
                               (blockIdx.x * BLOCK + threadIdx.x) & ~63u, true, (64u * (u32)out_stride) >> 4);
}

__host__ __device__ __forceinline__ bool fanout_owns(uint64_t out_stride) { return owns_slots(out_stride); }

#if CZ_KPART_HAS(1) || CZ_KPART_HAS(2)
__global__ __launch_bounds__(BLOCK) void k_zero_pad(uint8_t *__restrict__ out, uint64_t stride, uint32_t count,
                                                    uint32_t from)
{
    static_assert(BLOCK * 16 == 4096, "one chunk per workgroup trip");
    const uint64_t pad = stride - from;
    const uint64_t per = (pad + 4095u) / 4096u;
    const uint64_t total = per * count;
    for (uint64_t c = blockIdx.x; c < total; c += gridDim.x) {
        const uint64_t i = c / per, o = (c % per) * 4096u + 16u * threadIdx.x;
        if (o >= pad)
            continue;
        uint8_t *p = out + i * stride + from + o;
        const uint64_t nb = pad - o;
        if (nb >= 16u)
            reinterpret_cast<U16ua *>(p)->v = make_uint4(0u, 0u, 0u, 0u);
        else
            for (u32 b = 0; b < (u32)nb; b++)
                p[b] = 0;
    }
}

static void zero_pad_launch(const Launch &l, void *out, uint64_t stride, uint32_t count, hipStream_t s)
{
    if (l.pad_from != PAD_NONE)
        hipLaunchKernelGGL(k_zero_pad, dim3(pad_grid(stride, count, l.pad_from)), dim3(BLOCK), 0, s, (uint8_t *)out,
                           stride, count, (uint32_t)l.pad_from);
}
#endif

template <int ST, bool PAIR>
__global__ __launch_bounds__(BLOCK) CZ_OCC CZ_OPEN_UNI_OCC void k_seal_fanout_runs(
    const cz_fanout_run *__restrict__ runs, const cz_fanout_wave *__restrict__ waves, uint32_t nwaves,
    const uint8_t *__restrict__ in, const cz_fanout_sub *__restrict__ subs, const uint8_t *__restrict__ subkeys,
    uint8_t *__restrict__ out, uint32_t region_part16)
{
    const u32 w = __builtin_amdgcn_readfirstlane(blockIdx.x * WAVES + (threadIdx.x >> 6));
    if (w >= nwaves)
        return;
    const cz_fanout_wave wv = waves[w];
    const cz_fanout_run r = runs[wv.run];
    const uint8_t *payload = in + r.payload_off;
    uint8_t *o = out + r.out_off;
    bool staged = r.count >= 64u && ((((uintptr_t)payload | (uintptr_t)o | r.out_stride) & 15u) == 0);
    if constexpr (ST == ST_LINES)
        staged = staged && r.out_stride % 128 == 0 && r.len + 33u >= LINES_BYTES_MIN && r.out_stride < LINES_STRIDE_MAX;
    else if constexpr (ST == ST_REGION)
        staged = staged && 64 * r.out_stride <= REGION_MAX && ((64 * r.out_stride) >> 4) <= region_part16;
    seal_fanout_wave<ST, PAIR>(payload, r.len, r.flags, subs + r.first_sub, subkeys, o, r.out_stride, r.count,
                               fanout_owns(r.out_stride) ? 1 : 0, wv.first, staged, region_part16);
}

#if CZ_KPART_HAS(3)
__global__ __launch_bounds__(BLOCK) void k_seal_desc(const cz_frame_desc *__restrict__ desc,
                                                      const uint32_t *__restrict__ order, uint32_t count,
                                                      const uint8_t *__restrict__ in, uint8_t *__restrict__ out,
                                                      const uint8_t *__restrict__ subkeys)
{
    const uint32_t t = blockIdx.x * BLOCK + threadIdx.x;
    if (t >= count)
        return;
    const uint32_t i = order ? order[t] : t;
    const cz_frame_desc d = desc[i];
    u32 key[8];
    load_key(subkeys + 32ull * d.key_idx, key);
    const uint8_t *src = in + d.in_off;
    uint8_t *dst = out + d.out_off;
    if (aligned16(src, dst)) {
        EmitDirect<true> em{dst, d.len + 33u};
        seal_frame<MODE_ZMQ, true, EmitDirect<true>, false, false, false>(src, d.len, d.flags & 0xffu, d.counter, key, em);
    } else {
        EmitDirect<false> em{dst, d.len + 33u};
        seal_frame<MODE_ZMQ, false, EmitDirect<false>, false, false, false>(src, d.len, d.flags & 0xffu, d.counter, key, em);
    }
}

__global__ __launch_bounds__(BLOCK) void k_open_desc(const cz_frame_desc *__restrict__ desc,
                                                      const uint32_t *__restrict__ order, uint32_t count,
                                                      const uint8_t *__restrict__ in, uint8_t *__restrict__ out,
                                                      const uint8_t *__restrict__ subkeys,
                                                      uint16_t *__restrict__ status, uint64_t *__restrict__ nonces)
{
    const uint32_t t = blockIdx.x * BLOCK + threadIdx.x;
    if (t >= count)
        return;
    const uint32_t i = order ? order[t] : t;
    const cz_frame_desc d = desc[i];
    u32 key[8];
    load_key(subkeys + 32ull * d.key_idx, key);
    long long floor = (long long)d.counter;
    if (d.prev >= 0) {
        const cz_frame_desc p = desc[d.prev];
        floor = (long long)read_be64(in + p.in_off + 8);
    }
    const bool check = (d.flags & CZ_DESC_CHECK_NONCE) != 0;
    const uint8_t *src = in + d.in_off;
    uint8_t *dst = out + d.out_off;
    u32 fl = 0;
    u64 nonce = 0;
    u32 st;
    const u32 nout = d.len >= 33u ? d.len - 33u : 0u;
    if (aligned16(src, dst)) {
        EmitDirect<true> em{dst, nout};
        st = open_frame<MODE_ZMQ, true, EmitDirect<true>, false, false, false>(src, d.len, key, check, floor, &fl, &nonce, 0, em);
    } else {
        EmitDirect<false> em{dst, nout};
        st = open_frame<MODE_ZMQ, false, EmitDirect<false>, false, false, false>(src, d.len, key, check, floor, &fl, &nonce, 0, em);
    }
    status[i] = (uint16_t)(st | (st == CZ_STATUS_OK ? (fl << 8) : 0u));
    if (nonces)
        nonces[i] = nonce;
}

#endif

#ifdef CZ_DIAG_CLOCK
template <int ST, bool PAIR, int INA>
__device__ __forceinline__ void open_uniform_body(const uint8_t *__restrict__ in, uint64_t in_stride,
                                                  uint8_t *__restrict__ out, uint64_t out_stride, uint32_t count,
                                                  uint32_t size, const uint8_t *__restrict__ subkey, uint64_t floor0,
                                                  int check, uint16_t *__restrict__ status, int allow_un0, int prev0)
#else
template <int ST, bool PAIR, int INA = 16>
__global__ __launch_bounds__(BLOCK) CZ_OCC CZ_OPEN_UNI_OCC void k_open_uniform(const uint8_t *__restrict__ in, uint64_t in_stride,
                                                         uint8_t *__restrict__ out, uint64_t out_stride,
                                                         uint32_t count, uint32_t size,
                                                         const uint8_t *__restrict__ subkey, uint64_t floor0,
                                                         int check, uint16_t *__restrict__ status, int allow_un0,
                                                         int prev0 = 0)
#endif
{
    static_assert(INA == 16 || ST != ST_DIRECT, "unaligned bodies: staged plaintext only");
    extern __shared__ uint4 smem[];
    uint32_t i = blockIdx.x * BLOCK + threadIdx.x;
    if constexpr (ST == ST_SHIFT) {
        if (blockIdx.x * BLOCK + BLOCK <= count)
            i = blockIdx.x * BLOCK + class_permute(((uintptr_t)(out + (uint64_t)i * out_stride) & 64u) != 0,
                                                   reinterpret_cast<u32 *>(smem));
    }
    const uint32_t wave_first = (blockIdx.x * BLOCK + threadIdx.x) & ~63u;
    if (wave_first >= count)
        return;
    u32 key[8];
    load_key(subkey, key);
    const bool full_wave = wave_first + 64u <= count;
    const uint8_t *src = in + (uint64_t)i * in_stride;
    uint8_t *dst = out + (uint64_t)i * out_stride;
    const u32 nout = size >= 33u ? size - 33u : 0u;
    u32 fl = 0;
    u64 nonce = 0;
    u32 st;
// ... 1115 lines not shown
```

Baseline: 1924 GiB/s.

## Add hand-scheduled Salsa20 frame core asm starting at round two with scalar inputs

Adds a generated inline-asm Salsa20 core for the uniform-nonce frame path. It precomputes more of the frame-invariant second-round state per frame (x11 and two rotations) and feeds frame-invariant words as SGPR operands. It also uses lazy xor-pending tracking with v_xad/v_bitop3 fusion. This is meant to cut per-block VALU work in the seal keystream, and it is enabled for PAIR shift-lines paths except when INA==1. The cost is opaque hand-written asm, higher maintenance, and risk of register-pressure or scheduling regressions versus the compiler.

```diff
diff --git a/jeromq_amd/build.py b/jeromq_amd/build.py
--- a/jeromq_amd/build.py
+++ b/jeromq_amd/build.py
@@ -13,7 +13,7 @@
 LIB = os.environ.get("CZ_LIB_OUT", PRODUCT_LIB)
 SOURCES = ["cz_kernels.hip#1", "cz_kernels.hip#2", "cz_kernels.hip#3", "cz_x25519.hip", "cz_host.cpp", "cz_mechanism.cpp", "cz_wire.cpp", "cz_engine.cpp", "cz_handshake.cpp", "cz_curve_hs.cpp", "cz_hs_parse.cpp", "cz_acceptor.cpp", "cz_connector.cpp"]
 HEADERS = ["cz_accept.h", "cz_accept_kernels.h", "cz_connect.h", "cz_connect_kernels.h", "cz_hs_batch.h", "cz_hs_dev.h",
-           "cz_hs_records.h", "cz_hs_parse.h", "cz_device.h", "cz_fe25519.h", "cz_diag.h", "cz_dispatch.h", "cz_internal.h", "cz_launch.h", "cz_salsa_lazy.h", "cz_salsa_tail.h", "cz_session.h", os.path.join("..", "..", "include", "curvezmq_mi355x.h")]
+           "cz_hs_records.h", "cz_hs_parse.h", "cz_device.h", "cz_fe25519.h", "cz_diag.h", "cz_dispatch.h", "cz_internal.h", "cz_launch.h", "cz_salsa_frame.h", "cz_salsa_lazy.h", "cz_salsa_tail.h", "cz_session.h", os.path.join("..", "..", "include", "curvezmq_mi355x.h")]
 ARCH = os.environ.get("CZ_OFFLOAD_ARCH", "gfx950")
 LLVM_BIN = "/opt/rocm/lib/llvm/bin"
 BUNDLE_MAGIC = b"__CLANG_OFFLOAD_BUNDLE__"
diff --git a/jeromq_amd/csrc/cz_device.h b/jeromq_amd/csrc/cz_device.h
--- a/jeromq_amd/csrc/cz_device.h
+++ b/jeromq_amd/csrc/cz_device.h
@@ -2,6 +2,7 @@
 #include <hip/hip_runtime.h>
 #include <stdint.h>
 
+#include "cz_salsa_frame.h"
 #include "cz_salsa_lazy.h"
 #include "cz_salsa_tail.h"
 
@@ -136,16 +137,78 @@
     }
 }
 
-__device__ __forceinline__ void salsa20_block_frame(u32 x[16], const SalsaFrame &f, const u32 k[8], u32 n0, u32 n1,
-                                                    u32 c0)
+struct SalsaFrameR2 {
+    u32 x11;
+    u32 r8;
+    u32 r12;
+};
+
+__device__ __forceinline__ SalsaFrameR2 salsa_frame_r2(const SalsaFrame &f)
+{
+    SalsaFrameR2 g;
+    g.x11 = f.w[11] ^ srotl<7>(f.w[10] + f.w[9]);
+    g.r8 = rotl(g.x11 + f.w[10], 9);
+    g.r12 = rotl(f.w[15] + f.w[14], 7);
+    return g;
+}
+
+__device__ __forceinline__ void frame_core_entry(u32 e[16], const SalsaFrame &f, const SalsaFrameR2 &g, u32 c0,
+                                                 const u32 k[8])
+{
+#if CZ_FRAME_FIRST_ROUND == 3
+    rounds12_frame(e, f, c0, k);
+    (void)g;
+#else
+    static_assert(CZ_FRAME_FIRST_ROUND == 2 && CZ_FRAME_SCALAR_IN == 0x777fu && CZ_FRAME_ENTRY_PENDING == 0x1100u,
+                  "frame core entry");
+#pragma unroll
+    for (int i = 0; i < 16; i++)
+        e[i] = f.w[i];
+    e[0] = SIGMA0; e[4] = k[3]; e[8] = c0; e[12] = k[5];
+    e[4] ^= srotl<7>(e[0] + e[12]);  e[8] ^= srotl<9>(e[4] + e[0]);
+    e[12] ^= srotl<13>(e[8] + e[4]); e[0] ^= srotl<18>(e[12] + e[8]);
+    e[1] ^= srotl<7>(e[0] + e[3]);   e[2] ^= srotl<9>(e[1] + e[0]);
+    e[3] ^= srotl<13>(e[2] + e[1]);  e[0] ^= srotl<18>(e[3] + e[2]);
+    e[6] ^= srotl<7>(e[5] + e[4]);   e[7] ^= srotl<9>(e[6] + e[5]);
+    e[11] = g.x11;
+#endif
+}
+
+__device__ __forceinline__ constexpr bool frame_pending(int k) { return (CZ_FRAME_PENDING >> k) & 1u; }
+
+template <bool FRAME = true>
+__device__ __forceinline__ void salsa20_block_frame(u32 x[16], const SalsaFrame &f, const SalsaFrameR2 &g,
+                                                    const u32 k[8], u32 n0, u32 n1, u32 c0)
 {
     const u32 in[16] = {SIGMA0, k[0], k[1], k[2], k[3], SIGMA1, n0, n1, c0, 0u, SIGMA2, k[4], k[5], k[6], k[7], SIGMA3};
     u32 d[16];
-    rounds12_frame(x, f, c0, k);
-    rounds_lazy<true>(x, d);
-#pragma unroll
-    for (int i = 0; i < 16; i++)
-        x[i] = lazy_pending(i) ? ((x[i] ^ d[i]) + in[i]) : (x[i] + in[i]);
+    if constexpr (FRAME) {
+        u32 e[16], t0, t1, t2, t3;
+        frame_core_entry(e, f, g, c0, k);
+        asm(CZ_SALSA_FRAME_ASM
+            : "=&v"(x[0]), "=&v"(x[1]), "=&v"(x[2]), "=&v"(x[3]), "=&v"(x[4]), "=&v"(x[5]), "=&v"(x[6]), "=&v"(x[7]),
+              "=&v"(x[8]), "=&v"(x[9]), "=&v"(x[10]), "=&v"(x[11]), "=&v"(x[12]), "=&v"(x[13]), "=&v"(x[14]),
+              "=&v"(x[15]), "=&v"(d[0]), "=&v"(d[1]), "=&v"(d[2]), "=&v"(d[3]), "=&v"(d[4]), "=&v"(d[5]), "=&v"(d[6]),
+              "=&v"(d[7]), "=&v"(d[8]), "=&v"(d[9]), "=&v"(d[10]), "=&v"(d[11]), "=&v"(d[12]), "=&v"(d[13]),
+              "=&v"(d[14]), "=&v"(d[15]), "=&v"(t0), "=&v"(t1), "=&v"(t2), "=&v"(t3)
+            : CZ_FRAME_IN_0(e[0]), CZ_FRAME_IN_1(e[1]), CZ_FRAME_IN_2(e[2]), CZ_FRAME_IN_3(e[3]), CZ_FRAME_IN_4(e[4]),
+              CZ_FRAME_IN_5(e[5]), CZ_FRAME_IN_6(e[6]), CZ_FRAME_IN_7(e[7]), CZ_FRAME_IN_8(e[8]), CZ_FRAME_IN_9(e[9]),
+              CZ_FRAME_IN_10(e[10]), CZ_FRAME_IN_11(e[11]), CZ_FRAME_IN_12(e[12]), CZ_FRAME_IN_13(e[13]),
+              CZ_FRAME_IN_14(e[14]), CZ_FRAME_IN_15(e[15])
+#if CZ_FRAME_FIRST_ROUND == 2
+              , "v"(g.r8), "v"(g.r12)
+#endif
+        );
+#pragma unroll
+        for (int i = 0; i < 16; i++)
+            x[i] = frame_pending(i) ? ((x[i] ^ d[i]) + in[i]) : (x[i] + in[i]);
+    } else {
+        rounds12_frame(x, f, c0, k);
+        rounds_lazy<true>(x, d);
+#pragma unroll
+        for (int i = 0; i < 16; i++)
+            x[i] = lazy_pending(i) ? ((x[i] ^ d[i]) + in[i]) : (x[i] + in[i]);
+    }
 }
 
 __device__ __forceinline__ void tail_lazy(u32 x[16], u32 d[16])
diff --git a/jeromq_amd/csrc/cz_kernels.hip b/jeromq_amd/csrc/cz_kernels.hip
--- a/jeromq_amd/csrc/cz_kernels.hip
+++ b/jeromq_amd/csrc/cz_kernels.hip
@@ -460,7 +460,8 @@
 using EmitRegion = EmitRegionT<CZ_OPEN_STORE_CPOL>;
 using EmitRegionSeal = EmitRegionT<CZ_SEAL_STORE_CPOL == 2 ? 2 : 0>;
 
-template <int MODE, bool AL, class EM, bool PAIR = false, bool UN0 = false, bool LAZY = true, int INA = 16>
+template <int MODE, bool AL, class EM, bool PAIR = false, bool UN0 = false, bool LAZY = true, int INA = 16,
+          bool FRAME = true>
 __device__ __forceinline__ void seal_frame(const uint8_t *__restrict__ in0, u32 n, u32 flags, u64 counter,
                                            const u32 key[8], EM &em)
 {
@@ -500,11 +501,14 @@
         n0 = __builtin_amdgcn_readfirstlane(n0);
 
     [[maybe_unused]] SalsaFrame sf{};
+    [[maybe_unused]] SalsaFrameR2 sg{};
     if constexpr (UN0 && LAZY)
         sf = salsa_frame(key, n0, n1);
+    if constexpr (UN0 && LAZY && FRAME && PAIR)
+        sg = salsa_frame_r2(sf);
     auto ksblock = [&](u32 *xs, u32 c0, u32 c1) {
         if constexpr (UN0 && LAZY)
-            salsa20_block_frame(xs, sf, key, n0, n1, c0);
+            salsa20_block_frame<FRAME && PAIR>(xs, sf, sg, key, n0, n1, c0);
         else
             salsa20_block<LAZY>(xs, key, n0, n1, c0, c1);
     };
@@ -882,7 +886,7 @@
         sf = salsa_frame(key, n0, n1);
     auto ksblock = [&](u32 *xs, u32 c0, u32 c1) {
         if constexpr (UN0 && LAZY)
-            salsa20_block_frame(xs, sf, key, n0, n1, c0);
+            salsa20_block_frame<false>(xs, sf, SalsaFrameR2{}, key, n0, n1, c0);
         else
             salsa20_block<LAZY>(xs, key, n0, n1, c0, c1);
     };
@@ -2129,18 +2133,20 @@
             em.init_uniform(i - blockIdx.x * BLOCK, (u32)out_stride, out + (uint64_t)blockIdx.x * BLOCK * out_stride);
             const bool b2b = out_stride == (uint64_t)mlen && (mlen & 63u) != 0u;
             em.init_ext(b2b && i > 0u, b2b && i + 1u < count);
+            constexpr bool FRAME = !(PAIR && INA == 1);
             if (un0 && !em.mixed) {
                 if (__builtin_amdgcn_readfirstlane((((u32)(uintptr_t)dst & 64u) == 0u) ? 1u : 0u)) {
                     EmitShiftLinesUniClassSeal<1> ec{em};
-                    seal_frame<MODE, true, EmitShiftLinesUniClassSeal<1>, PAIR, true, true, INA>(src, len, fl,
-                                                                                               counter0 + i, key, ec);
+                    seal_frame<MODE, true, EmitShiftLinesUniClassSeal<1>, PAIR, true, true, INA, FRAME>(
+                        src, len, fl, counter0 + i, key, ec);
                 } else {
                     EmitShiftLinesUniClassSeal<0> ec{em};
-                    seal_frame<MODE, true, EmitShiftLinesUniClassSeal<0>, PAIR, true, true, INA>(src, len, fl,
-                                                                                               counter0 + i, key, ec);
+                    seal_frame<MODE, true, EmitShiftLinesUniClassSeal<0>, PAIR, true, true, INA, FRAME>(
+                        src, len, fl, counter0 + i, key, ec);
                 }
             } else if (un0)
-                seal_frame<MODE, true, EmitShiftLinesUniSeal, PAIR, true, true, INA>(src, len, fl, counter0 + i, key, em);
+                seal_frame<MODE, true, EmitShiftLinesUniSeal, PAIR, true, true, INA, FRAME>(src, len, fl, counter0 + i, key,
+                                                                                            em);
             else
                 seal_frame<MODE, true, EmitShiftLinesUniSeal, PAIR, false, true, INA>(src, len, fl, counter0 + i, key, em);
         } else {
diff --git a/jeromq_amd/csrc/cz_salsa_frame.h b/jeromq_amd/csrc/cz_salsa_frame.h
--- /dev/null
+++ b/jeromq_amd/csrc/cz_salsa_frame.h
@@ -0,0 +1,777 @@
+#pragma once
+#define CZ_FRAME_PENDING 0xde7bu
+#define CZ_FRAME_FIRST_ROUND 2
+#define CZ_FRAME_SCALAR_IN 0x777fu
+#define CZ_FRAME_ENTRY_PENDING 0x1100u
+#define CZ_FRAME_IN_0 "s"
+#define CZ_FRAME_IN_1 "s"
+#define CZ_FRAME_IN_2 "s"
+#define CZ_FRAME_IN_3 "s"
+#define CZ_FRAME_IN_4 "s"
+#define CZ_FRAME_IN_5 "s"
+#define CZ_FRAME_IN_6 "s"
+#define CZ_FRAME_IN_7 "v"
+#define CZ_FRAME_IN_8 "s"
+#define CZ_FRAME_IN_9 "s"
+#define CZ_FRAME_IN_10 "s"
+#define CZ_FRAME_IN_11 "v"
+#define CZ_FRAME_IN_12 "s"
+#define CZ_FRAME_IN_13 "s"
+#define CZ_FRAME_IN_14 "s"
+#define CZ_FRAME_IN_15 "v"
+#define CZ_SALSA_FRAME_ASM \
+    "v_xor_b32 %8, %44, %52\n" \
+    "v_xor_b32 %12, %48, %53\n" \
+    "v_add_u32 %35, %12, %51\n" \
+    "v_alignbit_b32 %35, %35, %35, 23\n" \
+    "v_xor_b32 %13, %49, %35\n" \
+    "v_add_u32 %20, %42, %43\n" \
+    "v_add_u32 %25, %8, %47\n" \
+    "v_add_u32 %30, %13, %12\n" \
+    "v_alignbit_b32 %20, %20, %20, 19\n" \
+    "v_alignbit_b32 %25, %25, %25, 19\n" \
+    "v_alignbit_b32 %30, %30, %30, 19\n" \
+    "v_xad_u32 %33, %40, %20, %43\n" \
+    "v_xad_u32 %34, %45, %25, %8\n" \
+    "v_xad_u32 %31, %50, %30, %13\n" \
+    "v_alignbit_b32 %33, %33, %33, 14\n" \
+    "v_alignbit_b32 %34, %34, %34, 14\n" \
+    "v_alignbit_b32 %31, %31, %31, 14\n" \
+    "v_xor_b32 %5, %41, %33\n" \
+    "v_xor_b32 %10, %46, %34\n" \
+    "v_add_u32 %32, %36, %12\n" \
+    "v_add_u32 %33, %37, %5\n" \
+    "v_add_u32 %34, %42, %10\n" \
+    "v_xad_u32 %35, %51, %31, %47\n" \
+    "v_alignbit_b32 %32, %32, %32, 25\n" \
+    "v_alignbit_b32 %33, %33, %33, 25\n" \
+    "v_alignbit_b32 %34, %34, %34, 25\n" \
+    "v_alignbit_b32 %35, %35, %35, 25\n" \
+    "v_bitop3_b32 %4, %40, %20, %32 bitop3:0x96\n" \
+    "v_bitop3_b32 %9, %45, %25, %33 bitop3:0x96\n" \
+    "v_bitop3_b32 %14, %50, %30, %34 bitop3:0x96\n" \
+    "v_xor_b32 %3, %39, %35\n" \
+    "v_add_u32 %24, %36, %4\n" \
+    "v_add_u32 %33, %9, %5\n" \
+    "v_add_u32 %18, %14, %10\n" \
+    "v_xad_u32 %23, %51, %31, %3\n" \
+    "v_alignbit_b32 %24, %24, %24, 23\n" \
+    "v_alignbit_b32 %33, %33, %33, 23\n" \
+    "v_alignbit_b32 %18, %18, %18, 23\n" \
+    "v_alignbit_b32 %23, %23, %23, 23\n" \
+    "v_xor_b32 %13, %13, %33\n" \
+    "v_xad_u32 %32, %8, %24, %4\n" \
+    "v_add_u32 %17, %13, %9\n" \
+    "v_xad_u32 %34, %38, %18, %14\n" \
+    "v_xad_u32 %35, %43, %23, %3\n" \
+    "v_alignbit_b32 %32, %32, %32, 19\n" \
+    "v_alignbit_b32 %17, %17, %17, 19\n" \
+    "v_alignbit_b32 %34, %34, %34, 19\n" \
+    "v_alignbit_b32 %35, %35, %35, 19\n" \
+    "v_xor_b32 %12, %12, %32\n" \
+    "v_xor_b32 %6, %42, %34\n" \
+    "v_xor_b32 %11, %47, %35\n" \
+    "v_xad_u32 %16, %8, %24, %12\n" \
+    "v_xad_u32 %21, %37, %17, %13\n" \
+    "v_xad_u32 %26, %38, %18, %6\n" \
+    "v_xad_u32 %35, %43, %23, %11\n" \
+    "v_alignbit_b32 %16, %16, %16, 14\n" \
+    "v_alignbit_b32 %21, %21, %21, 14\n" \
+    "v_alignbit_b32 %26, %26, %26, 14\n" \
+    "v_alignbit_b32 %35, %35, %35, 14\n" \
+    "v_bitop3_b32 %15, %51, %31, %35 bitop3:0x96\n" \
+    "v_xor_b32 %5, %5, %21\n" \
+    "v_xad_u32 %32, %36, %16, %3\n" \
+    "v_add_u32 %22, %5, %4\n" \
+    "v_xad_u32 %34, %10, %26, %9\n" \
+    "v_add_u32 %28, %15, %14\n" \
+    "v_alignbit_b32 %32, %32, %32, 25\n" \
+    "v_alignbit_b32 %22, %22, %22, 25\n" \
+    "v_alignbit_b32 %34, %34, %34, 25\n" \
+    "v_alignbit_b32 %28, %28, %28, 25\n" \
+    "v_bitop3_b32 %1, %37, %17, %32 bitop3:0x96\n" \
+    "v_xor_b32 %11, %11, %34\n" \
+    "v_xad_u32 %32, %36, %16, %1\n" \
+    "v_xad_u32 %33, %6, %22, %5\n" \
+    "v_xad_u32 %34, %10, %26, %11\n" \
+    "v_xad_u32 %35, %12, %28, %15\n" \
+    "v_alignbit_b32 %32, %32, %32, 23\n" \
+    "v_alignbit_b32 %33, %33, %33, 23\n" \
+    "v_alignbit_b32 %34, %34, %34, 23\n" \
+    "v_alignbit_b32 %35, %35, %35, 23\n" \
+    "v_bitop3_b32 %2, %38, %18, %32 bitop3:0x96\n" \
+    "v_bitop3_b32 %7, %43, %23, %33 bitop3:0x96\n" \
+    "v_bitop3_b32 %8, %8, %24, %34 bitop3:0x96\n" \
+    "v_xor_b32 %13, %13, %35\n" \
+    "v_add_u32 %19, %2, %1\n" \
+    "v_xad_u32 %20, %6, %22, %7\n" \
+    "v_add_u32 %25, %8, %11\n" \
+    "v_xad_u32 %30, %12, %28, %13\n" \
+    "v_alignbit_b32 %19, %19, %19, 19\n" \
+    "v_alignbit_b32 %20, %20, %20, 19\n" \
+    "v_alignbit_b32 %25, %25, %25, 19\n" \
+    "v_alignbit_b32 %30, %30, %30, 19\n" \
+    "v_xad_u32 %32, %3, %19, %2\n" \
+    "v_xad_u32 %21, %4, %20, %7\n" \
+    "v_xad_u32 %34, %9, %25, %8\n" \
+    "v_xad_u32 %31, %14, %30, %13\n" \
+    "v_alignbit_b32 %32, %32, %32, 14\n" \
+    "v_alignbit_b32 %21, %21, %21, 14\n" \
+    "v_alignbit_b32 %34, %34, %34, 14\n" \
+    "v_alignbit_b32 %31, %31, %31, 14\n" \
+    "v_bitop3_b32 %0, %36, %16, %32 bitop3:0x96\n" \
+    "v_bitop3_b32 %10, %10, %26, %34 bitop3:0x96\n" \
+    "v_xad_u32 %32, %12, %28, %0\n" \
+    "v_xad_u32 %33, %5, %21, %1\n" \
+    "v_xad_u32 %34, %6, %22, %10\n" \
+    "v_xad_u32 %35, %15, %31, %11\n" \
+    "v_alignbit_b32 %32, %32, %32, 25\n" \
+    "v_alignbit_b32 %33, %33, %33, 25\n" \
+    "v_alignbit_b32 %34, %34, %34, 25\n" \
+    "v_alignbit_b32 %35, %35, %35, 25\n" \
+    "v_bitop3_b32 %4, %4, %20, %32 bitop3:0x96\n" \
+    "v_bitop3_b32 %9, %9, %25, %33 bitop3:0x96\n" \
+    "v_bitop3_b32 %14, %14, %30, %34 bitop3:0x96\n" \
+    "v_bitop3_b32 %3, %3, %19, %35 bitop3:0x96\n" \
+    "v_add_u32 %24, %4, %0\n" \
+    "v_xad_u32 %33, %5, %21, %9\n" \
+    "v_add_u32 %18, %14, %10\n" \
+    "v_xad_u32 %35, %15, %31, %3\n" \
+    "v_alignbit_b32 %24, %24, %24, 23\n" \
+    "v_alignbit_b32 %33, %33, %33, 23\n" \
+    "v_alignbit_b32 %18, %18, %18, 23\n" \
+    "v_alignbit_b32 %35, %35, %35, 23\n" \
+    "v_xor_b32 %13, %13, %33\n" \
+    "v_xor_b32 %7, %7, %35\n" \
+    "v_xad_u32 %32, %8, %24, %4\n" \
+    "v_add_u32 %17, %13, %9\n" \
+    "v_xad_u32 %34, %2, %18, %14\n" \
+    "v_add_u32 %27, %7, %3\n" \
+    "v_alignbit_b32 %32, %32, %32, 19\n" \
+    "v_alignbit_b32 %17, %17, %17, 19\n" \
+    "v_alignbit_b32 %34, %34, %34, 19\n" \
+    "v_alignbit_b32 %27, %27, %27, 19\n" \
+    "v_bitop3_b32 %12, %12, %28, %32 bitop3:0x96\n" \
+    "v_bitop3_b32 %6, %6, %22, %34 bitop3:0x96\n" \
+    "v_xad_u32 %16, %8, %24, %12\n" \
+    "v_xad_u32 %33, %1, %17, %13\n" \
+    "v_xad_u32 %26, %2, %18, %6\n" \
+    "v_xad_u32 %35, %11, %27, %7\n" \
+    "v_alignbit_b32 %16, %16, %16, 14\n" \
+    "v_alignbit_b32 %33, %33, %33, 14\n" \
+    "v_alignbit_b32 %26, %26, %26, 14\n" \
+    "v_alignbit_b32 %35, %35, %35, 14\n" \
+    "v_bitop3_b32 %5, %5, %21, %33 bitop3:0x96\n" \
+    "v_bitop3_b32 %15, %15, %31, %35 bitop3:0x96\n" \
+    "v_xad_u32 %32, %0, %16, %3\n" \
+    "v_add_u32 %22, %5, %4\n" \
+    "v_xad_u32 %34, %10, %26, %9\n" \
+    "v_add_u32 %28, %15, %14\n" \
+    "v_alignbit_b32 %32, %32, %32, 25\n" \
+    "v_alignbit_b32 %22, %22, %22, 25\n" \
+    "v_alignbit_b32 %34, %34, %34, 25\n" \
+    "v_alignbit_b32 %28, %28, %28, 25\n" \
+    "v_bitop3_b32 %1, %1, %17, %32 bitop3:0x96\n" \
+    "v_bitop3_b32 %11, %11, %27, %34 bitop3:0x96\n" \
+    "v_xad_u32 %32, %0, %16, %1\n" \
+    "v_xad_u32 %33, %6, %22, %5\n" \
+    "v_xad_u32 %34, %10, %26, %11\n" \
+    "v_xad_u32 %35, %12, %28, %15\n" \
+    "v_alignbit_b32 %32, %32, %32, 23\n" \
+    "v_alignbit_b32 %33, %33, %33, 23\n" \
+    "v_alignbit_b32 %34, %34, %34, 23\n" \
+    "v_alignbit_b32 %35, %35, %35, 23\n" \
+    "v_bitop3_b32 %2, %2, %18, %32 bitop3:0x96\n" \
+    "v_xor_b32 %7, %7, %33\n" \
+    "v_bitop3_b32 %8, %8, %24, %34 bitop3:0x96\n" \
+    "v_xor_b32 %13, %13, %35\n" \
+    "v_add_u32 %19, %2, %1\n" \
+    "v_xad_u32 %20, %6, %22, %7\n" \
+    "v_add_u32 %25, %8, %11\n" \
+    "v_xad_u32 %30, %12, %28, %13\n" \
+    "v_alignbit_b32 %19, %19, %19, 19\n" \
+    "v_alignbit_b32 %20, %20, %20, 19\n" \
+    "v_alignbit_b32 %25, %25, %25, 19\n" \
+    "v_alignbit_b32 %30, %30, %30, 19\n" \
+    "v_xad_u32 %32, %3, %19, %2\n" \
+    "v_xad_u32 %21, %4, %20, %7\n" \
+    "v_xad_u32 %34, %9, %25, %8\n" \
+    "v_xad_u32 %31, %14, %30, %13\n" \
+    "v_alignbit_b32 %32, %32, %32, 14\n" \
+    "v_alignbit_b32 %21, %21, %21, 14\n" \
+    "v_alignbit_b32 %34, %34, %34, 14\n" \
+    "v_alignbit_b32 %31, %31, %31, 14\n" \
+    "v_bitop3_b32 %0, %0, %16, %32 bitop3:0x96\n" \
+    "v_bitop3_b32 %10, %10, %26, %34 bitop3:0x96\n" \
+    "v_xad_u32 %32, %12, %28, %0\n" \
+    "v_xad_u32 %33, %5, %21, %1\n" \
+    "v_xad_u32 %34, %6, %22, %10\n" \
+    "v_xad_u32 %35, %15, %31, %11\n" \
+    "v_alignbit_b32 %32, %32, %32, 25\n" \
+    "v_alignbit_b32 %33, %33, %33, 25\n" \
+    "v_alignbit_b32 %34, %34, %34, 25\n" \
+    "v_alignbit_b32 %35, %35, %35, 25\n" \
+    "v_bitop3_b32 %4, %4, %20, %32 bitop3:0x96\n" \
+    "v_bitop3_b32 %9, %9, %25, %33 bitop3:0x96\n" \
+    "v_bitop3_b32 %14, %14, %30, %34 bitop3:0x96\n" \
+    "v_bitop3_b32 %3, %3, %19, %35 bitop3:0x96\n" \
+    "v_add_u32 %24, %4, %0\n" \
+    "v_xad_u32 %29, %5, %21, %9\n" \
+    "v_add_u32 %18, %14, %10\n" \
+    "v_xad_u32 %23, %15, %31, %3\n" \
+    "v_alignbit_b32 %24, %24, %24, 23\n" \
+    "v_alignbit_b32 %29, %29, %29, 23\n" \
+    "v_alignbit_b32 %18, %18, %18, 23\n" \
+    "v_alignbit_b32 %23, %23, %23, 23\n" \
+    "v_xad_u32 %32, %8, %24, %4\n" \
+    "v_xad_u32 %33, %13, %29, %9\n" \
+    "v_xad_u32 %34, %2, %18, %14\n" \
+    "v_xad_u32 %35, %7, %23, %3\n" \
+    "v_alignbit_b32 %32, %32, %32, 19\n" \
+    "v_alignbit_b32 %33, %33, %33, 19\n" \
+    "v_alignbit_b32 %34, %34, %34, 19\n" \
+    "v_alignbit_b32 %35, %35, %35, 19\n" \
+    "v_bitop3_b32 %12, %12, %28, %32 bitop3:0x96\n" \
+    "v_xor_b32 %1, %1, %33\n" \
+    "v_bitop3_b32 %6, %6, %22, %34 bitop3:0x96\n" \
+    "v_xor_b32 %11, %11, %35\n" \
+    "v_xad_u32 %16, %8, %24, %12\n" \
+    "v_xad_u32 %33, %13, %29, %1\n" \
+    "v_xad_u32 %26, %2, %18, %6\n" \
+    "v_xad_u32 %35, %7, %23, %11\n" \
+    "v_alignbit_b32 %16, %16, %16, 14\n" \
+    "v_alignbit_b32 %33, %33, %33, 14\n" \
+    "v_alignbit_b32 %26, %26, %26, 14\n" \
+    "v_alignbit_b32 %35, %35, %35, 14\n" \
+    "v_bitop3_b32 %5, %5, %21, %33 bitop3:0x96\n" \
+    "v_bitop3_b32 %15, %15, %31, %35 bitop3:0x96\n" \
+    "v_xad_u32 %32, %0, %16, %3\n" \
+    "v_add_u32 %22, %5, %4\n" \
+    "v_xad_u32 %34, %10, %26, %9\n" \
+    "v_add_u32 %28, %15, %14\n" \
+    "v_alignbit_b32 %32, %32, %32, 25\n" \
+    "v_alignbit_b32 %22, %22, %22, 25\n" \
+    "v_alignbit_b32 %34, %34, %34, 25\n" \
+    "v_alignbit_b32 %28, %28, %28, 25\n" \
+    "v_xor_b32 %1, %1, %32\n" \
+    "v_xor_b32 %11, %11, %34\n" \
+    "v_xad_u32 %32, %0, %16, %1\n" \
+    "v_xad_u32 %33, %6, %22, %5\n" \
+    "v_xad_u32 %34, %10, %26, %11\n" \
+    "v_xad_u32 %35, %12, %28, %15\n" \
+    "v_alignbit_b32 %32, %32, %32, 23\n" \
+    "v_alignbit_b32 %33, %33, %33, 23\n" \
+    "v_alignbit_b32 %34, %34, %34, 23\n" \
+    "v_alignbit_b32 %35, %35, %35, 23\n" \
+    "v_bitop3_b32 %2, %2, %18, %32 bitop3:0x96\n" \
+    "v_bitop3_b32 %7, %7, %23, %33 bitop3:0x96\n" \
+    "v_bitop3_b32 %8, %8, %24, %34 bitop3:0x96\n" \
+    "v_bitop3_b32 %13, %13, %29, %35 bitop3:0x96\n" \
+    "v_add_u32 %19, %2, %1\n" \
+    "v_xad_u32 %20, %6, %22, %7\n" \
+    "v_add_u32 %25, %8, %11\n" \
+    "v_xad_u32 %30, %12, %28, %13\n" \
+    "v_alignbit_b32 %19, %19, %19, 19\n" \
+    "v_alignbit_b32 %20, %20, %20, 19\n" \
+    "v_alignbit_b32 %25, %25, %25, 19\n" \
+    "v_alignbit_b32 %30, %30, %30, 19\n" \
+    "v_xad_u32 %32, %3, %19, %2\n" \
+    "v_xad_u32 %21, %4, %20, %7\n" \
+    "v_xad_u32 %34, %9, %25, %8\n" \
+    "v_xad_u32 %31, %14, %30, %13\n" \
+    "v_alignbit_b32 %32, %32, %32, 14\n" \
+    "v_alignbit_b32 %21, %21, %21, 14\n" \
+    "v_alignbit_b32 %34, %34, %34, 14\n" \
+    "v_alignbit_b32 %31, %31, %31, 14\n" \
+    "v_bitop3_b32 %0, %0, %16, %32 bitop3:0x96\n" \
+    "v_bitop3_b32 %10, %10, %26, %34 bitop3:0x96\n" \
+    "v_xad_u32 %32, %12, %28, %0\n" \
+    "v_xad_u32 %33, %5, %21, %1\n" \
+    "v_xad_u32 %34, %6, %22, %10\n" \
+    "v_xad_u32 %35, %15, %31, %11\n" \
+    "v_alignbit_b32 %32, %32, %32, 25\n" \
+    "v_alignbit_b32 %33, %33, %33, 25\n" \
+    "v_alignbit_b32 %34, %34, %34, 25\n" \
+    "v_alignbit_b32 %35, %35, %35, 25\n" \
+    "v_bitop3_b32 %4, %4, %20, %32 bitop3:0x96\n" \
+    "v_bitop3_b32 %9, %9, %25, %33 bitop3:0x96\n" \
+    "v_bitop3_b32 %14, %14, %30, %34 bitop3:0x96\n" \
+    "v_bitop3_b32 %3, %3, %19, %35 bitop3:0x96\n" \
+    "v_add_u32 %24, %4, %0\n" \
+    "v_xad_u32 %29, %5, %21, %9\n" \
+    "v_add_u32 %18, %14, %10\n" \
+    "v_xad_u32 %23, %15, %31, %3\n" \
+    "v_alignbit_b32 %24, %24, %24, 23\n" \
+    "v_alignbit_b32 %29, %29, %29, 23\n" \
+    "v_alignbit_b32 %18, %18, %18, 23\n" \
+    "v_alignbit_b32 %23, %23, %23, 23\n" \
+    "v_xad_u32 %32, %8, %24, %4\n" \
+    "v_xad_u32 %33, %13, %29, %9\n" \
+    "v_xad_u32 %34, %2, %18, %14\n" \
+    "v_xad_u32 %35, %7, %23, %3\n" \
+    "v_alignbit_b32 %32, %32, %32, 19\n" \
+    "v_alignbit_b32 %33, %33, %33, 19\n" \
+    "v_alignbit_b32 %34, %34, %34, 19\n" \
+    "v_alignbit_b32 %35, %35, %35, 19\n" \
+    "v_bitop3_b32 %12, %12, %28, %32 bitop3:0x96\n" \
+    "v_xor_b32 %1, %1, %33\n" \
+    "v_bitop3_b32 %6, %6, %22, %34 bitop3:0x96\n" \
+    "v_xor_b32 %11, %11, %35\n" \
+    "v_xad_u32 %16, %8, %24, %12\n" \
+    "v_xad_u32 %33, %13, %29, %1\n" \
+    "v_xad_u32 %26, %2, %18, %6\n" \
+    "v_xad_u32 %35, %7, %23, %11\n" \
+    "v_alignbit_b32 %16, %16, %16, 14\n" \
+    "v_alignbit_b32 %33, %33, %33, 14\n" \
+    "v_alignbit_b32 %26, %26, %26, 14\n" \
+    "v_alignbit_b32 %35, %35, %35, 14\n" \
+    "v_bitop3_b32 %5, %5, %21, %33 bitop3:0x96\n" \
+    "v_bitop3_b32 %15, %15, %31, %35 bitop3:0x96\n" \
+    "v_xad_u32 %32, %0, %16, %3\n" \
+    "v_add_u32 %22, %5, %4\n" \
+    "v_xad_u32 %34, %10, %26, %9\n" \
+    "v_add_u32 %28, %15, %14\n" \
+    "v_alignbit_b32 %32, %32, %32, 25\n" \
+    "v_alignbit_b32 %22, %22, %22, 25\n" \
+    "v_alignbit_b32 %34, %34, %34, 25\n" \
+    "v_alignbit_b32 %28, %28, %28, 25\n" \
+    "v_xor_b32 %1, %1, %32\n" \
+    "v_xor_b32 %11, %11, %34\n" \
+    "v_xad_u32 %32, %0, %16, %1\n" \
+    "v_xad_u32 %33, %6, %22, %5\n" \
+    "v_xad_u32 %34, %10, %26, %11\n" \
+    "v_xad_u32 %35, %12, %28, %15\n" \
+    "v_alignbit_b32 %32, %32, %32, 23\n" \
+    "v_alignbit_b32 %33, %33, %33, 23\n" \
+    "v_alignbit_b32 %34, %34, %34, 23\n" \
+    "v_alignbit_b32 %35, %35, %35, 23\n" \
+    "v_bitop3_b32 %2, %2, %18, %32 bitop3:0x96\n" \
+    "v_bitop3_b32 %7, %7, %23, %33 bitop3:0x96\n" \
+    "v_bitop3_b32 %8, %8, %24, %34 bitop3:0x96\n" \
+    "v_bitop3_b32 %13, %13, %29, %35 bitop3:0x96\n" \
+    "v_add_u32 %19, %2, %1\n" \
+    "v_xad_u32 %20, %6, %22, %7\n" \
+    "v_add_u32 %25, %8, %11\n" \
+    "v_xad_u32 %30, %12, %28, %13\n" \
+    "v_alignbit_b32 %19, %19, %19, 19\n" \
+    "v_alignbit_b32 %20, %20, %20, 19\n" \
+    "v_alignbit_b32 %25, %25, %25, 19\n" \
+    "v_alignbit_b32 %30, %30, %30, 19\n" \
+    "v_xad_u32 %32, %3, %19, %2\n" \
+    "v_xad_u32 %21, %4, %20, %7\n" \
+    "v_xad_u32 %34, %9, %25, %8\n" \
+    "v_xad_u32 %31, %14, %30, %13\n" \
+    "v_alignbit_b32 %32, %32, %32, 14\n" \
+    "v_alignbit_b32 %21, %21, %21, 14\n" \
+    "v_alignbit_b32 %34, %34, %34, 14\n" \
+    "v_alignbit_b32 %31, %31, %31, 14\n" \
+    "v_bitop3_b32 %0, %0, %16, %32 bitop3:0x96\n" \
+    "v_bitop3_b32 %10, %10, %26, %34 bitop3:0x96\n" \
+    "v_xad_u32 %32, %12, %28, %0\n" \
+    "v_xad_u32 %33, %5, %21, %1\n" \
+    "v_xad_u32 %34, %6, %22, %10\n" \
+    "v_xad_u32 %35, %15, %31, %11\n" \
+    "v_alignbit_b32 %32, %32, %32, 25\n" \
+    "v_alignbit_b32 %33, %33, %33, 25\n" \
+    "v_alignbit_b32 %34, %34, %34, 25\n" \
+    "v_alignbit_b32 %35, %35, %35, 25\n" \
+    "v_bitop3_b32 %4, %4, %20, %32 bitop3:0x96\n" \
+    "v_bitop3_b32 %9, %9, %25, %33 bitop3:0x96\n" \
+    "v_bitop3_b32 %14, %14, %30, %34 bitop3:0x96\n" \
+    "v_bitop3_b32 %3, %3, %19, %35 bitop3:0x96\n" \
+    "v_add_u32 %24, %4, %0\n" \
+    "v_xad_u32 %29, %5, %21, %9\n" \
+    "v_add_u32 %18, %14, %10\n" \
+    "v_xad_u32 %23, %15, %31, %3\n" \
+    "v_alignbit_b32 %24, %24, %24, 23\n" \
+    "v_alignbit_b32 %29, %29, %29, 23\n" \
+    "v_alignbit_b32 %18, %18, %18, 23\n" \
+    "v_alignbit_b32 %23, %23, %23, 23\n" \
+    "v_xad_u32 %32, %8, %24, %4\n" \
+    "v_xad_u32 %33, %13, %29, %9\n" \
+    "v_xad_u32 %34, %2, %18, %14\n" \
+    "v_xad_u32 %35, %7, %23, %3\n" \
+    "v_alignbit_b32 %32, %32, %32, 19\n" \
+    "v_alignbit_b32 %33, %33, %33, 19\n" \
+    "v_alignbit_b32 %34, %34, %34, 19\n" \
+    "v_alignbit_b32 %35, %35, %35, 19\n" \
+    "v_bitop3_b32 %12, %12, %28, %32 bitop3:0x96\n" \
+    "v_xor_b32 %1, %1, %33\n" \
+    "v_bitop3_b32 %6, %6, %22, %34 bitop3:0x96\n" \
+    "v_xor_b32 %11, %11, %35\n" \
+    "v_xad_u32 %16, %8, %24, %12\n" \
+    "v_xad_u32 %33, %13, %29, %1\n" \
+    "v_xad_u32 %26, %2, %18, %6\n" \
+    "v_xad_u32 %35, %7, %23, %11\n" \
+    "v_alignbit_b32 %16, %16, %16, 14\n" \
+    "v_alignbit_b32 %33, %33, %33, 14\n" \
+    "v_alignbit_b32 %26, %26, %26, 14\n" \
+    "v_alignbit_b32 %35, %35, %35, 14\n" \
+    "v_bitop3_b32 %5, %5, %21, %33 bitop3:0x96\n" \
+    "v_bitop3_b32 %15, %15, %31, %35 bitop3:0x96\n" \
+    "v_xad_u32 %32, %0, %16, %3\n" \
+    "v_add_u32 %22, %5, %4\n" \
+    "v_xad_u32 %34, %10, %26, %9\n" \
+    "v_add_u32 %28, %15, %14\n" \
+    "v_alignbit_b32 %32, %32, %32, 25\n" \
+    "v_alignbit_b32 %22, %22, %22, 25\n" \
+    "v_alignbit_b32 %34, %34, %34, 25\n" \
+    "v_alignbit_b32 %28, %28, %28, 25\n" \
+    "v_xor_b32 %1, %1, %32\n" \
+    "v_xor_b32 %11, %11, %34\n" \
+    "v_xad_u32 %32, %0, %16, %1\n" \
+    "v_xad_u32 %33, %6, %22, %5\n" \
+    "v_xad_u32 %34, %10, %26, %11\n" \
+    "v_xad_u32 %35, %12, %28, %15\n" \
+    "v_alignbit_b32 %32, %32, %32, 23\n" \
+    "v_alignbit_b32 %33, %33, %33, 23\n" \
+    "v_alignbit_b32 %34, %34, %34, 23\n" \
+    "v_alignbit_b32 %35, %35, %35, 23\n" \
+    "v_bitop3_b32 %2, %2, %18, %32 bitop3:0x96\n" \
+    "v_bitop3_b32 %7, %7, %23, %33 bitop3:0x96\n" \
+    "v_bitop3_b32 %8, %8, %24, %34 bitop3:0x96\n" \
+    "v_bitop3_b32 %13, %13, %29, %35 bitop3:0x96\n" \
+    "v_add_u32 %19, %2, %1\n" \
+    "v_xad_u32 %20, %6, %22, %7\n" \
+    "v_add_u32 %25, %8, %11\n" \
+    "v_xad_u32 %30, %12, %28, %13\n" \
+    "v_alignbit_b32 %19, %19, %19, 19\n" \
+    "v_alignbit_b32 %20, %20, %20, 19\n" \
+    "v_alignbit_b32 %25, %25, %25, 19\n" \
+    "v_alignbit_b32 %30, %30, %30, 19\n" \
+    "v_xad_u32 %32, %3, %19, %2\n" \
+    "v_xad_u32 %21, %4, %20, %7\n" \
+    "v_xad_u32 %34, %9, %25, %8\n" \
+    "v_xad_u32 %31, %14, %30, %13\n" \
+    "v_alignbit_b32 %32, %32, %32, 14\n" \
+    "v_alignbit_b32 %21, %21, %21, 14\n" \
+    "v_alignbit_b32 %34, %34, %34, 14\n" \
+    "v_alignbit_b32 %31, %31, %31, 14\n" \
+    "v_bitop3_b32 %0, %0, %16, %32 bitop3:0x96\n" \
+    "v_bitop3_b32 %10, %10, %26, %34 bitop3:0x96\n" \
+    "v_xad_u32 %32, %12, %28, %0\n" \
+    "v_xad_u32 %33, %5, %21, %1\n" \
+    "v_xad_u32 %34, %6, %22, %10\n" \
+    "v_xad_u32 %35, %15, %31, %11\n" \
+    "v_alignbit_b32 %32, %32, %32, 25\n" \
+    "v_alignbit_b32 %33, %33, %33, 25\n" \
+    "v_alignbit_b32 %34, %34, %34, 25\n" \
+    "v_alignbit_b32 %35, %35, %35, 25\n" \
+    "v_bitop3_b32 %4, %4, %20, %32 bitop3:0x96\n" \
+    "v_bitop3_b32 %9, %9, %25, %33 bitop3:0x96\n" \
+    "v_bitop3_b32 %14, %14, %30, %34 bitop3:0x96\n" \
+    "v_bitop3_b32 %3, %3, %19, %35 bitop3:0x96\n" \
+    "v_add_u32 %24, %4, %0\n" \
+    "v_xad_u32 %33, %5, %21, %9\n" \
+    "v_add_u32 %18, %14, %10\n" \
+    "v_xad_u32 %35, %15, %31, %3\n" \
+    "v_alignbit_b32 %24, %24, %24, 23\n" \
+    "v_alignbit_b32 %33, %33, %33, 23\n" \
+    "v_alignbit_b32 %18, %18, %18, 23\n" \
+    "v_alignbit_b32 %35, %35, %35, 23\n" \
+    "v_xor_b32 %13, %13, %33\n" \
+    "v_xor_b32 %7, %7, %35\n" \
+    "v_xad_u32 %32, %8, %24, %4\n" \
+    "v_add_u32 %17, %13, %9\n" \
+    "v_xad_u32 %34, %2, %18, %14\n" \
+    "v_add_u32 %27, %7, %3\n" \
+    "v_alignbit_b32 %32, %32, %32, 19\n" \
+    "v_alignbit_b32 %17, %17, %17, 19\n" \
+    "v_alignbit_b32 %34, %34, %34, 19\n" \
+    "v_alignbit_b32 %27, %27, %27, 19\n" \
+    "v_bitop3_b32 %12, %12, %28, %32 bitop3:0x96\n" \
+    "v_bitop3_b32 %6, %6, %22, %34 bitop3:0x96\n" \
+    "v_xad_u32 %16, %8, %24, %12\n" \
+    "v_xad_u32 %33, %1, %17, %13\n" \
+    "v_xad_u32 %26, %2, %18, %6\n" \
+    "v_xad_u32 %35, %11, %27, %7\n" \
+    "v_alignbit_b32 %16, %16, %16, 14\n" \
+    "v_alignbit_b32 %33, %33, %33, 14\n" \
+    "v_alignbit_b32 %26, %26, %26, 14\n" \
+    "v_alignbit_b32 %35, %35, %35, 14\n" \
+    "v_bitop3_b32 %5, %5, %21, %33 bitop3:0x96\n" \
+    "v_bitop3_b32 %15, %15, %31, %35 bitop3:0x96\n" \
+    "v_xad_u32 %32, %0, %16, %3\n" \
+    "v_add_u32 %22, %5, %4\n" \
+    "v_xad_u32 %34, %10, %26, %9\n" \
+    "v_add_u32 %28, %15, %14\n" \
+    "v_alignbit_b32 %32, %32, %32, 25\n" \
+    "v_alignbit_b32 %22, %22, %22, 25\n" \
+    "v_alignbit_b32 %34, %34, %34, 25\n" \
+    "v_alignbit_b32 %28, %28, %28, 25\n" \
+    "v_bitop3_b32 %1, %1, %17, %32 bitop3:0x96\n" \
+    "v_bitop3_b32 %11, %11, %27, %34 bitop3:0x96\n" \
+    "v_xad_u32 %32, %0, %16, %1\n" \
+    "v_xad_u32 %33, %6, %22, %5\n" \
+    "v_xad_u32 %34, %10, %26, %11\n" \
+    "v_xad_u32 %35, %12, %28, %15\n" \
+    "v_alignbit_b32 %32, %32, %32, 23\n" \
+    "v_alignbit_b32 %33, %33, %33, 23\n" \
+    "v_alignbit_b32 %34, %34, %34, 23\n" \
+    "v_alignbit_b32 %35, %35, %35, 23\n" \
+    "v_bitop3_b32 %2, %2, %18, %32 bitop3:0x96\n" \
+    "v_xor_b32 %7, %7, %33\n" \
+    "v_bitop3_b32 %8, %8, %24, %34 bitop3:0x96\n" \
+    "v_xor_b32 %13, %13, %35\n" \
+    "v_add_u32 %19, %2, %1\n" \
+    "v_xad_u32 %20, %6, %22, %7\n" \
+    "v_add_u32 %25, %8, %11\n" \
+    "v_xad_u32 %30, %12, %28, %13\n" \
+    "v_alignbit_b32 %19, %19, %19, 19\n" \
+    "v_alignbit_b32 %20, %20, %20, 19\n" \
+    "v_alignbit_b32 %25, %25, %25, 19\n" \
+    "v_alignbit_b32 %30, %30, %30, 19\n" \
+    "v_xad_u32 %32, %3, %19, %2\n" \
+    "v_xad_u32 %21, %4, %20, %7\n" \
+    "v_xad_u32 %34, %9, %25, %8\n" \
+    "v_xad_u32 %31, %14, %30, %13\n" \
+    "v_alignbit_b32 %32, %32, %32, 14\n" \
+    "v_alignbit_b32 %21, %21, %21, 14\n" \
+    "v_alignbit_b32 %34, %34, %34, 14\n" \
+    "v_alignbit_b32 %31, %31, %31, 14\n" \
+    "v_bitop3_b32 %0, %0, %16, %32 bitop3:0x96\n" \
+    "v_bitop3_b32 %10, %10, %26, %34 bitop3:0x96\n" \
+    "v_xad_u32 %32, %12, %28, %0\n" \
+    "v_xad_u32 %33, %5, %21, %1\n" \
+    "v_xad_u32 %34, %6, %22, %10\n" \
+    "v_xad_u32 %35, %15, %31, %11\n" \
+    "v_alignbit_b32 %32, %32, %32, 25\n" \
+    "v_alignbit_b32 %33, %33, %33, 25\n" \
+    "v_alignbit_b32 %34, %34, %34, 25\n" \
+    "v_alignbit_b32 %35, %35, %35, 25\n" \
+    "v_bitop3_b32 %4, %4, %20, %32 bitop3:0x96\n" \
+    "v_bitop3_b32 %9, %9, %25, %33 bitop3:0x96\n" \
+    "v_bitop3_b32 %14, %14, %30, %34 bitop3:0x96\n" \
+    "v_bitop3_b32 %3, %3, %19, %35 bitop3:0x96\n" \
+    "v_add_u32 %24, %4, %0\n" \
+    "v_xad_u32 %33, %5, %21, %9\n" \
+    "v_add_u32 %18, %14, %10\n" \
+    "v_xad_u32 %23, %15, %31, %3\n" \
+    "v_alignbit_b32 %24, %24, %24, 23\n" \
+    "v_alignbit_b32 %33, %33, %33, 23\n" \
+    "v_alignbit_b32 %18, %18, %18, 23\n" \
+    "v_alignbit_b32 %23, %23, %23, 23\n" \
+    "v_xor_b32 %13, %13, %33\n" \
+    "v_xad_u32 %32, %8, %24, %4\n" \
+    "v_add_u32 %17, %13, %9\n" \
+    "v_xad_u32 %34, %2, %18, %14\n" \
+    "v_xad_u32 %35, %7, %23, %3\n" \
+    "v_alignbit_b32 %32, %32, %32, 19\n" \
+    "v_alignbit_b32 %17, %17, %17, 19\n" \
+    "v_alignbit_b32 %34, %34, %34, 19\n" \
+    "v_alignbit_b32 %35, %35, %35, 19\n" \
+    "v_bitop3_b32 %12, %12, %28, %32 bitop3:0x96\n" \
+    "v_bitop3_b32 %6, %6, %22, %34 bitop3:0x96\n" \
+    "v_xor_b32 %11, %11, %35\n" \
+    "v_xad_u32 %16, %8, %24, %12\n" \
+    "v_xad_u32 %33, %1, %17, %13\n" \
+    "v_xad_u32 %26, %2, %18, %6\n" \
+    "v_xad_u32 %35, %7, %23, %11\n" \
+    "v_alignbit_b32 %16, %16, %16, 14\n" \
+    "v_alignbit_b32 %33, %33, %33, 14\n" \
+    "v_alignbit_b32 %26, %26, %26, 14\n" \
+    "v_alignbit_b32 %35, %35, %35, 14\n" \
+    "v_bitop3_b32 %5, %5, %21, %33 bitop3:0x96\n" \
+    "v_bitop3_b32 %15, %15, %31, %35 bitop3:0x96\n" \
+    "v_xad_u32 %32, %0, %16, %3\n" \
+    "v_add_u32 %22, %5, %4\n" \
+    "v_xad_u32 %34, %10, %26, %9\n" \
+    "v_add_u32 %28, %15, %14\n" \
+    "v_alignbit_b32 %32, %32, %32, 25\n" \
+    "v_alignbit_b32 %22, %22, %22, 25\n" \
+    "v_alignbit_b32 %34, %34, %34, 25\n" \
+    "v_alignbit_b32 %28, %28, %28, 25\n" \
+    "v_bitop3_b32 %1, %1, %17, %32 bitop3:0x96\n" \
+    "v_xor_b32 %11, %11, %34\n" \
+    "v_xad_u32 %32, %0, %16, %1\n" \
+    "v_xad_u32 %33, %6, %22, %5\n" \
+    "v_xad_u32 %34, %10, %26, %11\n" \
+    "v_xad_u32 %35, %12, %28, %15\n" \
+    "v_alignbit_b32 %32, %32, %32, 23\n" \
+    "v_alignbit_b32 %33, %33, %33, 23\n" \
+    "v_alignbit_b32 %34, %34, %34, 23\n" \
+    "v_alignbit_b32 %35, %35, %35, 23\n" \
+    "v_bitop3_b32 %2, %2, %18, %32 bitop3:0x96\n" \
+    "v_bitop3_b32 %7, %7, %23, %33 bitop3:0x96\n" \
+    "v_bitop3_b32 %8, %8, %24, %34 bitop3:0x96\n" \
+    "v_xor_b32 %13, %13, %35\n" \
+    "v_add_u32 %19, %2, %1\n" \
+    "v_xad_u32 %20, %6, %22, %7\n" \
+    "v_add_u32 %25, %8, %11\n" \
+    "v_xad_u32 %30, %12, %28, %13\n" \
+    "v_alignbit_b32 %19, %19, %19, 19\n" \
+    "v_alignbit_b32 %20, %20, %20, 19\n" \
+    "v_alignbit_b32 %25, %25, %25, 19\n" \
+    "v_alignbit_b32 %30, %30, %30, 19\n" \
+    "v_xad_u32 %32, %3, %19, %2\n" \
+    "v_xad_u32 %21, %4, %20, %7\n" \
+    "v_xad_u32 %34, %9, %25, %8\n" \
+    "v_xad_u32 %31, %14, %30, %13\n" \
+    "v_alignbit_b32 %32, %32, %32, 14\n" \
+    "v_alignbit_b32 %21, %21, %21, 14\n" \
+    "v_alignbit_b32 %34, %34, %34, 14\n" \
+    "v_alignbit_b32 %31, %31, %31, 14\n" \
+    "v_bitop3_b32 %0, %0, %16, %32 bitop3:0x96\n" \
+    "v_bitop3_b32 %10, %10, %26, %34 bitop3:0x96\n" \
+    "v_xad_u32 %32, %12, %28, %0\n" \
+    "v_xad_u32 %33, %5, %21, %1\n" \
+    "v_xad_u32 %34, %6, %22, %10\n" \
+    "v_xad_u32 %35, %15, %31, %11\n" \
+    "v_alignbit_b32 %32, %32, %32, 25\n" \
+    "v_alignbit_b32 %33, %33, %33, 25\n" \
+    "v_alignbit_b32 %34, %34, %34, 25\n" \
+    "v_alignbit_b32 %35, %35, %35, 25\n" \
+    "v_bitop3_b32 %4, %4, %20, %32 bitop3:0x96\n" \
+    "v_bitop3_b32 %9, %9, %25, %33 bitop3:0x96\n" \
+    "v_bitop3_b32 %14, %14, %30, %34 bitop3:0x96\n" \
+    "v_bitop3_b32 %3, %3, %19, %35 bitop3:0x96\n" \
+    "v_add_u32 %24, %4, %0\n" \
+    "v_xad_u32 %29, %5, %21, %9\n" \
+    "v_add_u32 %18, %14, %10\n" \
+    "v_xad_u32 %35, %15, %31, %3\n" \
+    "v_alignbit_b32 %24, %24, %24, 23\n" \
+    "v_alignbit_b32 %29, %29, %29, 23\n" \
+    "v_alignbit_b32 %18, %18, %18, 23\n" \
+    "v_alignbit_b32 %35, %35, %35, 23\n" \
+    "v_xor_b32 %7, %7, %35\n" \
+    "v_xad_u32 %32, %8, %24, %4\n" \
+    "v_xad_u32 %33, %13, %29, %9\n" \
+    "v_xad_u32 %34, %2, %18, %14\n" \
+    "v_add_u32 %27, %7, %3\n" \
+    "v_alignbit_b32 %32, %32, %32, 19\n" \
+    "v_alignbit_b32 %33, %33, %33, 19\n" \
+    "v_alignbit_b32 %34, %34, %34, 19\n" \
+    "v_alignbit_b32 %27, %27, %27, 19\n" \
+    "v_bitop3_b32 %12, %12, %28, %32 bitop3:0x96\n" \
+    "v_xor_b32 %1, %1, %33\n" \
+    "v_bitop3_b32 %6, %6, %22, %34 bitop3:0x96\n" \
+    "v_xad_u32 %16, %8, %24, %12\n" \
+    "v_xad_u32 %33, %13, %29, %1\n" \
+    "v_xad_u32 %26, %2, %18, %6\n" \
+    "v_xad_u32 %35, %11, %27, %7\n" \
+    "v_alignbit_b32 %16, %16, %16, 14\n" \
+    "v_alignbit_b32 %33, %33, %33, 14\n" \
+    "v_alignbit_b32 %26, %26, %26, 14\n" \
+    "v_alignbit_b32 %35, %35, %35, 14\n" \
+    "v_bitop3_b32 %5, %5, %21, %33 bitop3:0x96\n" \
+    "v_bitop3_b32 %15, %15, %31, %35 bitop3:0x96\n" \
+    "v_xad_u32 %32, %0, %16, %3\n" \
+    "v_add_u32 %22, %5, %4\n" \
+    "v_xad_u32 %34, %10, %26, %9\n" \
+    "v_add_u32 %28, %15, %14\n" \
+    "v_alignbit_b32 %32, %32, %32, 25\n" \
+    "v_alignbit_b32 %22, %22, %22, 25\n" \
+    "v_alignbit_b32 %34, %34, %34, 25\n" \
+    "v_alignbit_b32 %28, %28, %28, 25\n" \
+    "v_xor_b32 %1, %1, %32\n" \
+    "v_bitop3_b32 %11, %11, %27, %34 bitop3:0x96\n" \
+    "v_xad_u32 %32, %0, %16, %1\n" \
+    "v_xad_u32 %33, %6, %22, %5\n" \
+    "v_xad_u32 %34, %10, %26, %11\n" \
+    "v_xad_u32 %35, %12, %28, %15\n" \
+    "v_alignbit_b32 %32, %32, %32, 23\n" \
+    "v_alignbit_b32 %33, %33, %33, 23\n" \
+    "v_alignbit_b32 %34, %34, %34, 23\n" \
+    "v_alignbit_b32 %35, %35, %35, 23\n" \
+    "v_bitop3_b32 %2, %2, %18, %32 bitop3:0x96\n" \
+    "v_xor_b32 %7, %7, %33\n" \
+    "v_bitop3_b32 %8, %8, %24, %34 bitop3:0x96\n" \
+    "v_bitop3_b32 %13, %13, %29, %35 bitop3:0x96\n" \
+    "v_add_u32 %19, %2, %1\n" \
+    "v_xad_u32 %20, %6, %22, %7\n" \
+    "v_add_u32 %25, %8, %11\n" \
+    "v_xad_u32 %30, %12, %28, %13\n" \
+    "v_alignbit_b32 %19, %19, %19, 19\n" \
+    "v_alignbit_b32 %20, %20, %20, 19\n" \
+    "v_alignbit_b32 %25, %25, %25, 19\n" \
+    "v_alignbit_b32 %30, %30, %30, 19\n" \
+    "v_xad_u32 %32, %3, %19, %2\n" \
+    "v_xad_u32 %21, %4, %20, %7\n" \
+    "v_xad_u32 %34, %9, %25, %8\n" \
+    "v_xad_u32 %31, %14, %30, %13\n" \
+    "v_alignbit_b32 %32, %32, %32, 14\n" \
+    "v_alignbit_b32 %21, %21, %21, 14\n" \
+    "v_alignbit_b32 %34, %34, %34, 14\n" \
+    "v_alignbit_b32 %31, %31, %31, 14\n" \
+    "v_bitop3_b32 %0, %0, %16, %32 bitop3:0x96\n" \
+    "v_bitop3_b32 %10, %10, %26, %34 bitop3:0x96\n" \
+    "v_xad_u32 %32, %12, %28, %0\n" \
+    "v_xad_u32 %33, %5, %21, %1\n" \
+    "v_xad_u32 %34, %6, %22, %10\n" \
+    "v_xad_u32 %35, %15, %31, %11\n" \
+    "v_alignbit_b32 %32, %32, %32, 25\n" \
+    "v_alignbit_b32 %33, %33, %33, 25\n" \
+    "v_alignbit_b32 %34, %34, %34, 25\n" \
+    "v_alignbit_b32 %35, %35, %35, 25\n" \
+    "v_bitop3_b32 %4, %4, %20, %32 bitop3:0x96\n" \
+    "v_bitop3_b32 %9, %9, %25, %33 bitop3:0x96\n" \
+    "v_bitop3_b32 %14, %14, %30, %34 bitop3:0x96\n" \
+    "v_bitop3_b32 %3, %3, %19, %35 bitop3:0x96\n" \
+    "v_add_u32 %24, %4, %0\n" \
+    "v_xad_u32 %29, %5, %21, %9\n" \
+    "v_add_u32 %18, %14, %10\n" \
+    "v_xad_u32 %23, %15, %31, %3\n" \
+    "v_alignbit_b32 %24, %24, %24, 23\n" \
+    "v_alignbit_b32 %29, %29, %29, 23\n" \
+    "v_alignbit_b32 %18, %18, %18, 23\n" \
+    "v_alignbit_b32 %23, %23, %23, 23\n" \
+    "v_xad_u32 %32, %8, %24, %4\n" \
+    "v_xad_u32 %33, %13, %29, %9\n" \
+    "v_xad_u32 %34, %2, %18, %14\n" \
+    "v_xad_u32 %35, %7, %23, %3\n" \
+    "v_alignbit_b32 %32, %32, %32, 19\n" \
+    "v_alignbit_b32 %33, %33, %33, 19\n" \
+    "v_alignbit_b32 %34, %34, %34, 19\n" \
+    "v_alignbit_b32 %35, %35, %35, 19\n" \
+    "v_bitop3_b32 %12, %12, %28, %32 bitop3:0x96\n" \
+    "v_xor_b32 %1, %1, %33\n" \
+    "v_bitop3_b32 %6, %6, %22, %34 bitop3:0x96\n" \
+    "v_xor_b32 %11, %11, %35\n" \
+    "v_xad_u32 %16, %8, %24, %12\n" \
+    "v_xad_u32 %33, %13, %29, %1\n" \
+    "v_xad_u32 %34, %2, %18, %6\n" \
+    "v_xad_u32 %35, %7, %23, %11\n" \
+    "v_alignbit_b32 %16, %16, %16, 14\n" \
+    "v_alignbit_b32 %33, %33, %33, 14\n" \
+    "v_alignbit_b32 %34, %34, %34, 14\n" \
+    "v_alignbit_b32 %35, %35, %35, 14\n" \
+    "v_bitop3_b32 %5, %5, %21, %33 bitop3:0x96\n" \
+    "v_xor_b32 %10, %10, %34\n" \
+    "v_bitop3_b32 %15, %15, %31, %35 bitop3:0x96\n" \
+    "v_xor_b32 %0, %0, %16\n" \
+    "v_add_u32 %17, %0, %3\n" \
+    "v_add_u32 %22, %5, %4\n" \
+    "v_add_u32 %27, %10, %9\n" \
+    "v_add_u32 %28, %15, %14\n" \
+    "v_alignbit_b32 %17, %17, %17, 25\n" \
+    "v_alignbit_b32 %22, %22, %22, 25\n" \
+    "v_alignbit_b32 %27, %27, %27, 25\n" \
+    "v_alignbit_b32 %28, %28, %28, 25\n" \
+    "v_xad_u32 %32, %1, %17, %0\n" \
+    "v_xad_u32 %33, %6, %22, %5\n" \
+    "v_xad_u32 %34, %11, %27, %10\n" \
+    "v_xad_u32 %35, %12, %28, %15\n" \
+    "v_alignbit_b32 %32, %32, %32, 23\n" \
+    "v_alignbit_b32 %33, %33, %33, 23\n" \
+    "v_alignbit_b32 %34, %34, %34, 23\n" \
+    "v_alignbit_b32 %35, %35, %35, 23\n" \
+    "v_bitop3_b32 %2, %2, %18, %32 bitop3:0x96\n" \
+    "v_bitop3_b32 %7, %7, %23, %33 bitop3:0x96\n" \
+    "v_bitop3_b32 %8, %8, %24, %34 bitop3:0x96\n" \
+    "v_bitop3_b32 %13, %13, %29, %35 bitop3:0x96\n" \
+    "v_xad_u32 %19, %1, %17, %2\n" \
+    "v_xad_u32 %20, %6, %22, %7\n" \
+    "v_xad_u32 %25, %11, %27, %8\n" \
+    "v_xad_u32 %30, %12, %28, %13\n" \
+    "v_alignbit_b32 %19, %19, %19, 19\n" \
+    "v_alignbit_b32 %20, %20, %20, 19\n" \
+    "v_alignbit_b32 %25, %25, %25, 19\n" \
+    "v_alignbit_b32 %30, %30, %30, 19\n" \
+    "v_xad_u32 %16, %3, %19, %2\n" \
+    "v_xad_u32 %21, %4, %20, %7\n" \
+    "v_xad_u32 %26, %9, %25, %8\n" \
+    "v_xad_u32 %31, %14, %30, %13\n" \
+    "v_alignbit_b32 %16, %16, %16, 14\n" \
+    "v_alignbit_b32 %21, %21, %21, 14\n" \
+    "v_alignbit_b32 %26, %26, %26, 14\n" \
+    "v_alignbit_b32 %31, %31, %31, 14\n"
```

Result: no change. 1925 GiB/s (median of 6 runs) (+0.0%).
